# TUMFTM/CamRaDepth

Hardware: AMD Instinct MI355X
Metric: training images/sec at 256x416 bf16 (higher is better)
Workload: dtype bf16; 1 GPU; CamRaDepth base (image+radar) train step, 8x7x256x416 per GPU, bf16 MFMA / fp32 accumulate, diffGradNorm + OneCycleLR, Dropout2d/DropPath on; global_batch=8, parallelism=dp1, hip_graph=True

## Files before the change

camradepth_amd/csrc/norm.hip:

```cpp
#include <stdlib.h>
#include "common.h"

namespace {

constexpr int TPB = 256;
constexpr int U = 4;

struct Map {
  int cg, pl, PL; bool active;
  __device__ Map(int C) {
    int CG = C >> 3;
    PL = TPB / CG;
    if (PL < 1) PL = 1;
    active = threadIdx.x < PL * CG;
    cg = threadIdx.x % CG;
    pl = threadIdx.x / CG;
  }
};

__device__ __forceinline__ void fold_rows(float* sm, int n, int rows) {
  for (int i = threadIdx.x; i < n; i += TPB) {
    float a = sm[i];
    for (int r = 1; r < rows; ++r) a += sm[(long long)r * n + i];
    sm[i] = a;
  }
  __syncthreads();
}

template <int XF>
__global__ __launch_bounds__(TPB) void k_gn_stats(const void* x, int x_f32, int x_ld, long long P, int C, int chunk,
                                                  crd_sum_t* stats, crd_sum_t* chan) {
  extern __shared__ float sm[];
  const int b = blockIdx.y;
  Map m(C);
  float s[8], ss[8];
#pragma unroll
  for (int j = 0; j < 8; ++j) s[j] = ss[j] = 0.f;
  if (m.active) {
    long long p0 = (long long)blockIdx.x * chunk, p1 = p0 + chunk;
    if (p1 > P) p1 = P;
    for (long long p = p0 + m.pl; p < p1; p += (long long)U * m.PL) {
      float v[U][8];
#pragma unroll
      for (int u = 0; u < U; ++u) {
        long long pp = p + (long long)u * m.PL;
        if (pp >= p1) pp = p1 - 1;
        load8t<XF>(x, ((long long)b * P + pp) * x_ld + m.cg * 8, v[u]);
      }
#pragma unroll
      for (int u = 0; u < U; ++u)
        if (p + (long long)u * m.PL < p1) {
#pragma unroll
          for (int j = 0; j < 8; ++j) { s[j] += v[u][j]; ss[j] += v[u][j] * v[u][j]; }
        }
    }
    float4* row = reinterpret_cast<float4*>(sm + (long long)m.pl * 2 * C + m.cg * 16);
#pragma unroll
    for (int j = 0; j < 4; ++j) row[j] = make_float4(s[2 * j], ss[2 * j], s[2 * j + 1], ss[2 * j + 1]);
  }
  __syncthreads();
  fold_rows(sm, 2 * C, m.PL);
  if (chan)
    for (int i = threadIdx.x; i < 2 * C; i += TPB) stat_add(&chan[(long long)b * C * 2 + i], sm[i]);
  if (stats)
    for (int g = threadIdx.x; g < (C >> 4) * 2; g += TPB) {
      int slab = g >> 1, which = g & 1;
      float a = 0.f;
#pragma unroll
      for (int j = 0; j < 16; ++j) a += sm[(slab * 16 + j) * 2 + which];
      stat_add(&stats[((long long)b * (C >> 4) + slab) * 2 + which], a);
    }
}

__global__ __launch_bounds__(TPB) void k_attn_out_residual_stats(const float* x, const float* u, const float* S, const float* bp,
                                                                 const float* dp, long long P, int C, int chunk, float* x1,
                                                                 crd_sum_t* stats) {
  extern __shared__ float sm[];
  const int b = blockIdx.y;
  Map m(C);
  if (m.active) {
    float s[8], ss[8], uu[8], bb[8];
#pragma unroll
    for (int j = 0; j < 8; ++j) s[j] = ss[j] = 0.f;
    const float dps = dp ? dp[b] : 1.f;
    load8(u, (long long)b * C + m.cg * 8, 1, uu);
    load8(bp, m.cg * 8, 1, bb);
    long long p0 = (long long)blockIdx.x * chunk, p1 = p0 + chunk;
    if (p1 > P) p1 = P;
    for (long long p = p0 + m.pl; p < p1; p += (long long)U * m.PL) {
      float v[U][8], sv[U];
#pragma unroll
      for (int q = 0; q < U; ++q) {
        long long pp = p + (long long)q * m.PL;
        if (pp >= p1) pp = p1 - 1;
        load8(x, ((long long)b * P + pp) * C + m.cg * 8, 1, v[q]);
        sv[q] = S[(long long)b * P + pp];
      }
#pragma unroll
      for (int q = 0; q < U; ++q)
        if (p + (long long)q * m.PL < p1) {
#pragma unroll
          for (int j = 0; j < 8; ++j) {
            v[q][j] += dps * bf_round(uu[j] * sv[q] + bb[j]);
            s[j] += v[q][j]; ss[j] += v[q][j] * v[q][j];
          }
          store8_f32(x1, ((long long)b * P + p + (long long)q * m.PL) * C + m.cg * 8, v[q]);
        }
    }
    float4* row = reinterpret_cast<float4*>(sm + (long long)m.pl * 2 * C + m.cg * 16);
#pragma unroll
    for (int j = 0; j < 4; ++j) row[j] = make_float4(s[2 * j], ss[2 * j], s[2 * j + 1], ss[2 * j + 1]);
  }
  __syncthreads();
  fold_rows(sm, 2 * C, m.PL);
  for (int g = threadIdx.x; g < (C >> 4) * 2; g += TPB) {
    int slab = g >> 1, which = g & 1;
    float a = 0.f;
#pragma unroll
    for (int j = 0; j < 16; ++j) a += sm[(slab * 16 + j) * 2 + which];
    stat_add(&stats[((long long)b * (C >> 4) + slab) * 2 + which], a);
  }
}

template <int XF, int YF, int ACT>
__global__ __launch_bounds__(TPB) void k_gn_apply(const void* x, int x_f32, int x_ld, long long P, int C, int chunk,
                                                  const crd_sum_t* stats, int gmul, const float* gamma, const float* beta,
                                                  int act, const float* mask, void* y, int y_ld, int y_f32, float y_inv_scale,
                                                  void* y2, int y2_ld) {
  const int b = blockIdx.y;
  Map m(C);
  if (!m.active) return;
  const int c0 = m.cg * 8;
  long long p0 = (long long)blockIdx.x * chunk, p1 = p0 + chunk;
  if (p1 > P) p1 = P;
  long long p = p0 + m.pl;
  float v[U][8];
  auto load_batch = [&](long long q) {
#pragma unroll
    for (int u = 0; u < U; ++u) {
      long long pp = q + (long long)u * m.PL;
      if (pp >= p1) pp = p1 - 1;
      load8t<XF>(x, ((long long)b * P + pp) * x_ld + c0, v[u]);
    }
  };
  if (p < p1) load_batch(p);
  float ga[8], be[8], mk[8];
  load8(gamma, c0, 1, ga);
  load8(beta, c0, 1, be);
  if (mask) load8(mask, (long long)b * C + c0, 1, mk);
  else {
#pragma unroll
    for (int j = 0; j < 8; ++j) mk[j] = 1.f;
  }
  float mean, rstd;
  const int grp = (c0 >> 4) / gmul;
  gn_mean_rstd(stats + (long long)b * (C >> 4) * 2, grp * gmul, gmul, (float)P * 16.f * gmul, mean, rstd);
#pragma unroll
  for (int j = 0; j < 8; ++j) {
    ga[j] *= rstd;
    be[j] -= mean * ga[j];
  }
  for (bool first = true; p < p1; p += (long long)U * m.PL, first = false) {
    if (!first) load_batch(p);
#pragma unroll
    for (int u = 0; u < U; ++u) {
      const long long pp = p + (long long)u * m.PL;
      if (pp < p1) {
#pragma unroll
        for (int j = 0; j < 8; ++j) {
          float w = v[u][j] * ga[j] + be[j];
          if (ACT == 1) w = gelu_exact(w);
          v[u][j] = w * mk[j];
        }
        if (YF == 3) {
          store8_fp8(y, ((long long)b * P + pp) * y_ld + c0, v[u], y_inv_scale);
          store8_bf16(y2, ((long long)b * P + pp) * y2_ld + c0, v[u]);
        } else if (YF == 2) store8_fp8(y, ((long long)b * P + pp) * y_ld + c0, v[u], y_inv_scale);
        else if (YF) store8_f32(reinterpret_cast<float*>(y), ((long long)b * P + pp) * y_ld + c0, v[u]);
        else store8_bf16(y, ((long long)b * P + pp) * y_ld + c0, v[u]);
      }
    }
  }
}

template <int XF, int DF, int ACT>
__global__ __launch_bounds__(TPB) void k_gn_bwd_reduce(const void* x, int x_f32, int x_ld, const void* dy, int dy_f32,
                                                       int dy_ld, long long P, int C, int Cs, int chunk, const crd_sum_t* stats,
                                                       int gmul, const float* gamma, const float* beta, int act,
                                                       const float* mask, crd_sum_t* r, float* partial) {
  extern __shared__ float sm[];
  const int b = blockIdx.y, cs = blockIdx.z * Cs;
  Map m(Cs);
  if (m.active) {
    const int c0 = cs + m.cg * 8;
    long long p0 = (long long)blockIdx.x * chunk, p1 = p0 + chunk;
    if (p1 > P) p1 = P;
    long long p = p0 + m.pl;
    float v[U][8], d[U][8];
    auto load_batch = [&](long long q) {
#pragma unroll
      for (int u = 0; u < U; ++u) {
        long long pp = q + (long long)u * m.PL;
        if (pp >= p1) pp = p1 - 1;
        load8t<XF>(x, ((long long)b * P + pp) * x_ld + c0, v[u]);
        load8t<DF>(dy, ((long long)b * P + pp) * dy_ld + c0, d[u]);
      }
    };
    if (p < p1) load_batch(p);
    float ga[8], be[8], mk[8], s0[8], s1[8];
    load8(gamma, c0, 1, ga);
    load8(beta, c0, 1, be);
    if (mask) load8(mask, (long long)b * C + c0, 1, mk);
#pragma unroll
    for (int j = 0; j < 8; ++j) {
      if (!mask) mk[j] = 1.f;
      s0[j] = s1[j] = 0.f;
    }
    float mean, rstd;
    const int grp = (c0 >> 4) / gmul;
    gn_mean_rstd(stats + (long long)b * (C >> 4) * 2, grp * gmul, gmul, (float)P * 16.f * gmul, mean, rstd);
    for (bool first = true; p < p1; p += (long long)U * m.PL, first = false) {
      if (!first) load_batch(p);
#pragma unroll
      for (int u = 0; u < U; ++u)
        if (p + (long long)u * m.PL < p1) {
#pragma unroll
          for (int j = 0; j < 8; ++j) {
            float xh = (v[u][j] - mean) * rstd;
            float g = d[u][j] * mk[j];
            if (ACT == 1) g *= gelu_grad(xh * ga[j] + be[j]);
            s0[j] += g; s1[j] += g * xh;
          }
        }
    }
    float4* row = reinterpret_cast<float4*>(sm + (long long)m.pl * 2 * Cs + m.cg * 16);
#pragma unroll
    for (int j = 0; j < 4; ++j) row[j] = make_float4(s0[2 * j], s1[2 * j], s0[2 * j + 1], s1[2 * j + 1]);
  }
  __syncthreads();
  fold_rows(sm, 2 * Cs, m.PL);
  if (partial) {
    float* dst = partial + ((long long)b * gridDim.x + blockIdx.x) * 2 * C + cs * 2;
    for (int i = threadIdx.x; i < 2 * Cs; i += TPB) dst[i] = sm[i];
    return;
  }
  for (int i = threadIdx.x; i < 2 * Cs; i += TPB) {
    const float v = sm[i];
    grad_add(&r[((long long)b * C + cs) * 2 + i], v);
    sm[i] = v * gamma[cs + (i >> 1)];
  }
  __syncthreads();
  const int cpg = 16 * gmul, G = C / cpg, Gs = Cs / cpg;
  crd_sum_t* rg = r + (long long)gridDim.y * C * 2 + ((long long)b * G + cs / cpg) * 2;
  for (int gi = threadIdx.x; gi < 2 * Gs; gi += TPB) {
    const int grp = gi >> 1, which = gi & 1;
    float acc = 0.f;
    for (int c = grp * cpg; c < (grp + 1) * cpg; ++c) acc += sm[c * 2 + which];
    grad_add(&rg[grp * 2 + which], acc);
  }
}

__global__ __launch_bounds__(TPB) void k_gn_bwd_finalize(const float* partial, int nblk, int C, int gmul, const float* gamma,
                                                         crd_sum_t* r, int B) {
  __shared__ float sm[4][64][2];
  const int b = blockIdx.y, c = blockIdx.x * 64 + (threadIdx.x & 63), lane = threadIdx.x >> 6;
  float s0 = 0.f, s1 = 0.f;
  if (c < C)
    for (int k = lane; k < nblk; k += 4) {
      const float* p = partial + ((long long)b * nblk + k) * 2 * C + c * 2;
      s0 += p[0]; s1 += p[1];
    }
  sm[lane][threadIdx.x & 63][0] = s0; sm[lane][threadIdx.x & 63][1] = s1;
  __syncthreads();
  if (lane == 0 && c < C) {
    s0 = sm[0][threadIdx.x][0] + sm[1][threadIdx.x][0] + sm[2][threadIdx.x][0] + sm[3][threadIdx.x][0];
    s1 = sm[0][threadIdx.x][1] + sm[1][threadIdx.x][1] + sm[2][threadIdx.x][1] + sm[3][threadIdx.x][1];
    r[((long long)b * C + c) * 2] = to_fx(s0, GRAD_ONE);
    r[((long long)b * C + c) * 2 + 1] = to_fx(s1, GRAD_ONE);
    const float g = gamma[c];
    sm[0][threadIdx.x][0] = g * s0; sm[0][threadIdx.x][1] = g * s1;
  }
  __syncthreads();
  if (threadIdx.x < 8) {
    const int slab = threadIdx.x >> 1, which = threadIdx.x & 1, c0 = blockIdx.x * 64 + slab * 16;
    if (c0 < C) {
      float a = 0.f;
      for (int j = 0; j < 16; ++j) a += sm[0][slab * 16 + j][which];
      const int cpg = 16 * gmul;
      grad_add(r + (long long)B * C * 2 + ((long long)b * (C / cpg) + c0 / cpg) * 2 + which, a);
    }
  }
}

template <int XF, int DF, int ACT>
__global__ __launch_bounds__(TPB) void k_gn_bwd_apply(const void* x, int x_f32, int x_ld, const void* dy, int dy_f32,
                                                      int dy_ld, long long P, int C, int chunk, const crd_sum_t* stats,
                                                      int gmul, const float* gamma, const float* beta, int act,
                                                      const float* mask, const crd_sum_t* r, float* dgamma, float* dbeta,
                                                      void* dx, int dx_f32, int dx_ld, int dx_acc, int B, void* dx2, int dx2_ld,
                                                      const float* scale2, unsigned char* dx8, int dx8_ld, const float* scale8,
                                                      unsigned* amax8) {
  const int b = blockIdx.y;
  Map m(C);
  const int c0 = m.cg * 8;
  __shared__ float s_amax[TPB / 64];
  const float inv8 = (dx8 && scale8) ? 1.f / fmaxf(*scale8, 1e-30f) : 0.f;
  float amax = 0.f;
  long long p0 = (long long)blockIdx.x * chunk, p1 = p0 + chunk;
  if (p1 > P) p1 = P;
  long long p = p0 + m.pl;
  float v[U][8], d[U][8];
  auto load_batch = [&](long long q) {
#pragma unroll
    for (int u = 0; u < U; ++u) {
      long long pp = q + (long long)u * m.PL;
      if (pp >= p1) pp = p1 - 1;
      load8t<XF>(x, ((long long)b * P + pp) * x_ld + c0, v[u]);
      load8t<DF>(dy, ((long long)b * P + pp) * dy_ld + c0, d[u]);
    }
  };
  if (m.active && p < p1) load_batch(p);
  if (b == 0 && dgamma) {
    for (int c = blockIdx.x * TPB + threadIdx.x; c < C; c += gridDim.x * TPB) {
      const float ob = dbeta[c], og = dgamma[c];
      long long g0, g1;
      sum_samples(r, B, C, c, g0, g1);
      dbeta[c] = ob + (float)g0 * (1.f / GRAD_ONE);
      dgamma[c] = og + (float)g1 * (1.f / GRAD_ONE);
    }
  }
  if (!m.active && !amax8) return;
  if (m.active) {
  float ga[8], be[8], mk[8];
  load8(gamma, c0, 1, ga);
  load8(beta, c0, 1, be);
  if (mask) load8(mask, (long long)b * C + c0, 1, mk);
  else {
#pragma unroll
    for (int j = 0; j < 8; ++j) mk[j] = 1.f;
  }
  const int grp = (c0 >> 4) / gmul;
  const int cpg = 16 * gmul;
  const float inv_m = 1.f / ((float)P * cpg);
  const crd_sum_t* rg = r + (long long)B * C * 2 + ((long long)b * (C / cpg) + grp) * 2;
  const float S1 = grad_get(rg) * inv_m, S2 = grad_get(rg + 1) * inv_m;
  float mean, rstd;
  gn_mean_rstd(stats + (long long)b * (C >> 4) * 2, grp * gmul, gmul, (float)P * cpg, mean, rstd);
  const float sc2 = (dx2 && scale2) ? scale2[b] : 1.f;
  for (bool first = true; p < p1; p += (long long)U * m.PL, first = false) {
    if (!first) load_batch(p);
#pragma unroll
    for (int u = 0; u < U; ++u) {
      const long long pp = p + (long long)u * m.PL;
      if (pp >= p1) continue;
      float o[8];
#pragma unroll
      for (int j = 0; j < 8; ++j) {
        float xh = (v[u][j] - mean) * rstd;
        float g = d[u][j] * mk[j];
        if (ACT == 1) g *= gelu_grad(xh * ga[j] + be[j]);
        o[j] = (ga[j] * g - S1 - xh * S2) * rstd;
      }
      const long long off = ((long long)b * P + pp) * dx_ld + c0;
      if (dx_f32) {
        float* q = reinterpret_cast<float*>(dx);
        if (dx_acc) {
          float w[8];
          load8(dx, off, 1, w);
#pragma unroll
          for (int j = 0; j < 8; ++j) o[j] += w[j];
        }
        store8_f32(q, off, o);
      } else {
        if (dx_acc) {
          float w[8];
          load8(dx, off, 0, w);
#pragma unroll
          for (int j = 0; j < 8; ++j) o[j] += w[j];
        }
        store8_bf16(dx, off, o);
      }
      if (dx8) {
        const uint32_t w0 = pack_bf2(o[0], o[1]), w1 = pack_bf2(o[2], o[3]), w2 = pack_bf2(o[4], o[5]), w3 = pack_bf2(o[6], o[7]);
        const float r[8] = {bf_lo(w0), bf_hi(w0), bf_lo(w1), bf_hi(w1), bf_lo(w2), bf_hi(w2), bf_lo(w3), bf_hi(w3)};
        const float chk = ((r[0] + r[1]) + (r[2] + r[3])) + ((r[4] + r[5]) + (r[6] + r[7]));
        if (!(fabsf(chk) < 3.0e38f)) crd_tu_nonfinite = 1;
#pragma unroll
        for (int j = 0; j < 8; ++j) amax = fmaxf(amax, fabsf(r[j]));
        uint2 q8;
        q8.x = pack_fp8x4(r[0] * inv8, r[1] * inv8, r[2] * inv8, r[3] * inv8);
        q8.y = pack_fp8x4(r[4] * inv8, r[5] * inv8, r[6] * inv8, r[7] * inv8);
        *reinterpret_cast<uint2*>(dx8 + ((long long)b * P + pp) * dx8_ld + c0) = q8;
      }
      if (dx2) {
#pragma unroll
        for (int j = 0; j < 8; ++j) o[j] *= sc2;
        store8_bf16(dx2, ((long long)b * P + pp) * dx2_ld + c0, o);
      }
    }
  }
  }
  if (amax8) {
#pragma unroll
    for (int o_ = 32; o_ > 0; o_ >>= 1) amax = fmaxf(amax, __shfl_xor(amax, o_));
    if ((threadIdx.x & 63) == 0) s_amax[threadIdx.x >> 6] = amax;
    __syncthreads();
    if (threadIdx.x == 0) {
      float a_ = s_amax[0];
      for (int w_ = 1; w_ < TPB / 64; ++w_) a_ = fmaxf(a_, s_amax[w_]);
      if (a_ > 0.f) atomicMax(amax8 + ((blockIdx.x + blockIdx.y * gridDim.x) % CRD_FP8_AMAX_SLOTS), __float_as_uint(a_));
    }
  }
}

inline void grid_for(long long P, int C, int B, dim3& grid, int& chunk, bool reduce = false) {
  int CG = C >> 3;
  int PL = TPB / CG; if (PL < 1) PL = 1;
  long long per_block = (long long)PL * 8;
  long long nblk = (P + per_block - 1) / per_block;
  static int minpix = -1, small = 256;
  if (minpix < 0) {
    minpix = crd_dev_int("CRD_GN_MINPIX", 2);
    small = crd_dev_int("CRD_GN_SMALL", 256);
  }
  if (nblk * B < small && minpix < 8) {
    per_block = (long long)PL * minpix;
    nblk = (P + per_block - 1) / per_block;
  }
  static int cap_r = -1, cap_e = -1;
  if (cap_r < 0) { cap_r = crd_dev_int("CRD_GN_CAP_R", 768); cap_e = crd_dev_int("CRD_GN_CAP_E", 4096); }
  long long cap = (reduce ? cap_r : cap_e) / (B > 0 ? B : 1); if (cap < 1) cap = 1;
  if (nblk > cap) nblk = cap;
  if (nblk < 1) nblk = 1;
  chunk = (int)((P + nblk - 1) / nblk);
  nblk = (P + chunk - 1) / chunk;
  grid = dim3((unsigned)nblk, (unsigned)B);
}

int check_common(const char* name, int x_ld, int x_coff, int C, int x_f32) {
  if (C % 16 != 0 || C > 2048) { crd_set_error("%s: C must be a multiple of 16 and <= 2048 (got %d)", name, C); return CRD_E_UNSUPPORTED; }
  if (x_ld % 8 || x_coff % 8) { crd_set_error("%s: ld/coff must be multiples of 8", name); return CRD_E_INVALID; }
  (void)x_f32;
  return CRD_OK;
}

inline size_t lds_rows(int C) {
  int PL = TPB / (C >> 3); if (PL < 1) PL = 1;
  return (size_t)PL * 2 * C * sizeof(float);
}

inline const void* off_ptr(const void* p, int f32, int coff) {
  return f32 ? (const void*)(reinterpret_cast<const float*>(p) + coff) : (const void*)(reinterpret_cast<const bf16_t*>(p) + coff);
}

}

extern "C" int crd_gn_stats(const void* x, int32_t x_f32, int32_t x_ld, int32_t x_coff, int32_t B, int32_t P, int32_t C,
                            crd_sum_t* stats, crd_sum_t* chan_sums, crd_stream_t stream) {
  CRD_CHECK_ARG(x && (stats || chan_sums), "crd_gn_stats: null pointer");
  int rc = check_common("crd_gn_stats", x_ld, x_coff, C, x_f32);
  if (rc) return rc;
  dim3 grid; int chunk;
  grid_for(P, C, B, grid, chunk, true);
  if (x_f32) hipLaunchKernelGGL(k_gn_stats<1>, grid, dim3(TPB), lds_rows(C), as_stream(stream), off_ptr(x, x_f32, x_coff),
                                x_f32, x_ld, (long long)P, C, chunk, stats, chan_sums);
  else hipLaunchKernelGGL(k_gn_stats<0>, grid, dim3(TPB), lds_rows(C), as_stream(stream), off_ptr(x, x_f32, x_coff),
                          x_f32, x_ld, (long long)P, C, chunk, stats, chan_sums);
  CRD_LAUNCH_CHECK("crd_gn_stats");
  return CRD_OK;
}

extern "C" int crd_attn_out_residual_stats(const float* x, const float* u, const float* S, const float* bp, const float* dp,
                                           int32_t B, int32_t N, int32_t C, float* x1, crd_sum_t* stats, crd_stream_t stream) {
  CRD_CHECK_ARG(x && u && S && bp && x1 && stats, "crd_attn_out_residual_stats: null pointer");
  int rc = check_common("crd_attn_out_residual_stats", C, 0, C, 1);
  if (rc) return rc;
  dim3 grid; int chunk;
  grid_for(N, C, B, grid, chunk, true);
  hipLaunchKernelGGL(k_attn_out_residual_stats, grid, dim3(TPB), lds_rows(C), as_stream(stream), x, u, S, bp, dp, (long long)N, C,
                     chunk, x1, stats);
  CRD_LAUNCH_CHECK("crd_attn_out_residual_stats");
  return CRD_OK;
}

extern "C" int crd_gn_apply(const void* x, int32_t x_f32, int32_t x_ld, int32_t x_coff, int32_t B, int32_t P, int32_t C,
                            const crd_sum_t* stats, int32_t gmul, const float* gamma, const float* beta, int32_t act,
                            const float* mask, void* y, int32_t y_f32, int32_t y_ld, int32_t y_coff, crd_stream_t stream) {
  CRD_CHECK_ARG(x && stats && gamma && beta && y, "crd_gn_apply: null pointer");
  CRD_CHECK_ARG(gmul >= 1 && (C / 16) % gmul == 0, "crd_gn_apply: bad gmul %d for C=%d", gmul, C);
  CRD_CHECK_ARG(y_ld % 8 == 0 && y_coff % 8 == 0, "crd_gn_apply: y_ld/y_coff must be multiples of 8");
  int rc = check_common("crd_gn_apply", x_ld, x_coff, C, x_f32);
  if (rc) return rc;
  dim3 grid; int chunk;
  grid_for(P, C, B, grid, chunk);
  void* yp = y_f32 ? (void*)(reinterpret_cast<float*>(y) + y_coff) : (void*)(reinterpret_cast<bf16_t*>(y) + y_coff);
#define CRD_GN_APPLY(XF, YF, ACT)                                                                                        \
  hipLaunchKernelGGL((k_gn_apply<XF, YF, ACT>), grid, dim3(TPB), 0, as_stream(stream), off_ptr(x, x_f32, x_coff), x_f32, \
                     x_ld, (long long)P, C, chunk, stats, gmul, gamma, beta, act, mask, yp, y_ld, y_f32, 1.f, nullptr, 0)
  const int key = (x_f32 ? 4 : 0) | (y_f32 ? 2 : 0) | (act ? 1 : 0);
  switch (key) {
    case 0: CRD_GN_APPLY(0, 0, 0); break;  case 1: CRD_GN_APPLY(0, 0, 1); break;
    case 2: CRD_GN_APPLY(0, 1, 0); break;  case 3: CRD_GN_APPLY(0, 1, 1); break;
    case 4: CRD_GN_APPLY(1, 0, 0); break;  case 5: CRD_GN_APPLY(1, 0, 1); break;
    case 6: CRD_GN_APPLY(1, 1, 0); break;  default: CRD_GN_APPLY(1, 1, 1); break;
  }
#undef CRD_GN_APPLY
  CRD_LAUNCH_CHECK("crd_gn_apply");
  return CRD_OK;
}

extern "C" int crd_gn_apply_fp8(const void* x, int32_t x_f32, int32_t x_ld, int32_t x_coff, int32_t B, int32_t P, int32_t C,
                                const crd_sum_t* stats, int32_t gmul, const float* gamma, const float* beta, int32_t act,
                                const float* mask, void* y_fp8, int32_t y_ld, int32_t y_coff, float y_scale, void* y_bf16,
                                int32_t yb_ld, int32_t yb_coff, crd_stream_t stream) {
  CRD_CHECK_ARG(x && stats && gamma && beta && y_fp8 && y_scale > 0.f, "crd_gn_apply_fp8: null pointer / bad scale");
  CRD_CHECK_ARG(gmul >= 1 && (C / 16) % gmul == 0, "crd_gn_apply_fp8: bad gmul %d for C=%d", gmul, C);
  CRD_CHECK_ARG(y_ld % 8 == 0 && y_coff % 8 == 0 && yb_ld % 8 == 0 && yb_coff % 8 == 0, "crd_gn_apply_fp8: ld/coff must be multiples of 8");
  int rc = check_common("crd_gn_apply_fp8", x_ld, x_coff, C, x_f32);
  if (rc) return rc;
  dim3 grid; int chunk;
  grid_for(P, C, B, grid, chunk);
  void* yp = reinterpret_cast<unsigned char*>(y_fp8) + y_coff;
  void* y2 = y_bf16 ? (void*)(reinterpret_cast<bf16_t*>(y_bf16) + yb_coff) : nullptr;
#define CRD_GN_APPLY8(XF, YF, ACT)                                                                                       \
  hipLaunchKernelGGL((k_gn_apply<XF, YF, ACT>), grid, dim3(TPB), 0, as_stream(stream), off_ptr(x, x_f32, x_coff), x_f32, \
                     x_ld, (long long)P, C, chunk, stats, gmul, gamma, beta, act, mask, yp, y_ld, 0, 1.f / y_scale, y2, yb_ld)
  switch ((x_f32 ? 4 : 0) | (y2 ? 2 : 0) | (act ? 1 : 0)) {
    case 0: CRD_GN_APPLY8(0, 2, 0); break;  case 1: CRD_GN_APPLY8(0, 2, 1); break;
    case 2: CRD_GN_APPLY8(0, 3, 0); break;  case 3: CRD_GN_APPLY8(0, 3, 1); break;
    case 4: CRD_GN_APPLY8(1, 2, 0); break;  case 5: CRD_GN_APPLY8(1, 2, 1); break;
    case 6: CRD_GN_APPLY8(1, 3, 0); break;  default: CRD_GN_APPLY8(1, 3, 1); break;
  }
#undef CRD_GN_APPLY8
  CRD_LAUNCH_CHECK("crd_gn_apply_fp8");
  return CRD_OK;
}

extern "C" int crd_gn_bwd_reduce(const void* x, int32_t x_f32, int32_t x_ld, int32_t x_coff, const void* dy, int32_t dy_f32,
                                 int32_t dy_ld, int32_t dy_coff, int32_t B, int32_t P, int32_t C, const crd_sum_t* stats,
                                 int32_t gmul, const float* gamma, const float* beta, int32_t act, const float* mask,
                                 crd_sum_t* r, float* scratch, int64_t scratch_capacity, crd_stream_t stream) {
  CRD_CHECK_ARG(x && dy && stats && gamma && beta && r, "crd_gn_bwd_reduce: null pointer");
  CRD_CHECK_ARG(gmul >= 1 && (C / 16) % gmul == 0, "crd_gn_bwd_reduce: bad gmul");
  CRD_CHECK_ARG(dy_ld % 8 == 0 && dy_coff % 8 == 0, "crd_gn_bwd_reduce: dy_ld/dy_coff must be multiples of 8");
  int rc = check_common("crd_gn_bwd_reduce", x_ld, x_coff, C, x_f32);
  if (rc) return rc;
  dim3 grid; int chunk;
  int S = 1;
  static int slicing = -1;
  if (slicing < 0) slicing = crd_dev_int("CRD_GN_RED_SLICES", 1);
  if (slicing && !scratch && C >= 256) {
    const int cpg = 16 * gmul;
    for (int s_ = 8; s_ > 1; s_ >>= 1)
      if (C % s_ == 0 && (C / s_) % cpg == 0 && (C / s_) % 8 == 0 && C / s_ >= 64) { S = s_; break; }
  }
  const int Cs = C / S;
  grid_for(P, Cs, B * S, grid, chunk, true);
  grid = dim3(grid.x, (unsigned)B, (unsigned)S);
  float* part = (scratch && (long long)B * grid.x * 2 * C <= scratch_capacity && grid.x > 1) ? scratch : nullptr;
#define CRD_GN_RED(XF, DF, ACT)                                                                                              \
  hipLaunchKernelGGL((k_gn_bwd_reduce<XF, DF, ACT>), grid, dim3(TPB), lds_rows(Cs), as_stream(stream),                     \
                     off_ptr(x, x_f32, x_coff), x_f32, x_ld, off_ptr(dy, dy_f32, dy_coff), dy_f32, dy_ld, (long long)P, C, \
                     Cs, chunk, stats, gmul, gamma, beta, act, mask, r, part)
  switch ((x_f32 ? 4 : 0) | (dy_f32 ? 2 : 0) | (act ? 1 : 0)) {
    case 0: CRD_GN_RED(0, 0, 0); break;  case 1: CRD_GN_RED(0, 0, 1); break;
    case 2: CRD_GN_RED(0, 1, 0); break;  case 3: CRD_GN_RED(0, 1, 1); break;
    case 4: CRD_GN_RED(1, 0, 0); break;  case 5: CRD_GN_RED(1, 0, 1); break;
    case 6: CRD_GN_RED(1, 1, 0); break;  default: CRD_GN_RED(1, 1, 1); break;
  }
#undef CRD_GN_RED
  if (part)
    hipLaunchKernelGGL(k_gn_bwd_finalize, dim3(cdiv(C, 64), B), dim3(TPB), 0, as_stream(stream), scratch, (int)grid.x, C, gmul,
                       gamma, r, B);
  CRD_LAUNCH_CHECK("crd_gn_bwd_reduce");
  return CRD_OK;
}

static int gn_bwd_apply_impl(const void* x, int32_t x_f32, int32_t x_ld, int32_t x_coff, const void* dy, int32_t dy_f32,
                             int32_t dy_ld, int32_t dy_coff, int32_t B, int32_t P, int32_t C, const crd_sum_t* stats,
                             int32_t gmul, const float* gamma, const float* beta, int32_t act, const float* mask,
                             const crd_sum_t* r, float* dgamma, float* dbeta, void* dx, int32_t dx_f32, int32_t dx_ld,
                             int32_t dx_coff, int32_t dx_accumulate, void* dx2, int32_t dx2_ld, const float* scale2,
                             void* dx8, int32_t dx8_ld, int32_t dx8_coff, const float* scale8, uint32_t* amax8, crd_stream_t stream) {
  unsigned char* dx8p = dx8 ? reinterpret_cast<unsigned char*>(dx8) + dx8_coff : nullptr;
  CRD_CHECK_ARG(x && dy && stats && gamma && beta && r && dx, "crd_gn_bwd_apply: null pointer");
  CRD_CHECK_ARG(!dx2 || dx2_ld % 8 == 0, "crd_gn_bwd_apply: dx2_ld must be a multiple of 8");
  CRD_CHECK_ARG((dgamma == nullptr) == (dbeta == nullptr), "crd_gn_bwd_apply: dgamma and dbeta go together");
  CRD_CHECK_ARG(gmul >= 1 && (C / 16) % gmul == 0, "crd_gn_bwd_apply: bad gmul");
  CRD_CHECK_ARG(dy_ld % 8 == 0 && dy_coff % 8 == 0 && dx_ld % 8 == 0 && dx_coff % 8 == 0,
                "crd_gn_bwd_apply: dy/dx ld/coff must be multiples of 8");
  int rc = check_common("crd_gn_bwd_apply", x_ld, x_coff, C, x_f32);
  if (rc) return rc;
  dim3 grid; int chunk;
  grid_for(P, C, B, grid, chunk);
  void* dxp = dx_f32 ? (void*)(reinterpret_cast<float*>(dx) + dx_coff) : (void*)(reinterpret_cast<bf16_t*>(dx) + dx_coff);
#define CRD_GN_BAP(XF, DF, ACT)                                                                                              \
  hipLaunchKernelGGL((k_gn_bwd_apply<XF, DF, ACT>), grid, dim3(TPB), 0, as_stream(stream), off_ptr(x, x_f32, x_coff), x_f32, \
                     x_ld, off_ptr(dy, dy_f32, dy_coff), dy_f32, dy_ld, (long long)P, C, chunk, stats, gmul, gamma, beta,  \
                     act, mask, r, dgamma, dbeta, dxp, dx_f32, dx_ld, dx_accumulate, B, dx2, dx2_ld, scale2, dx8p, dx8_ld, scale8,  \
                     amax8)
  switch ((x_f32 ? 4 : 0) | (dy_f32 ? 2 : 0) | (act ? 1 : 0)) {
    case 0: CRD_GN_BAP(0, 0, 0); break;  case 1: CRD_GN_BAP(0, 0, 1); break;
    case 2: CRD_GN_BAP(0, 1, 0); break;  case 3: CRD_GN_BAP(0, 1, 1); break;
    case 4: CRD_GN_BAP(1, 0, 0); break;  case 5: CRD_GN_BAP(1, 0, 1); break;
    case 6: CRD_GN_BAP(1, 1, 0); break;  default: CRD_GN_BAP(1, 1, 1); break;
  }
#undef CRD_GN_BAP
  CRD_LAUNCH_CHECK("crd_gn_bwd_apply");
  return CRD_OK;
}

extern "C" int crd_gn_bwd_apply(const void* x, int32_t x_f32, int32_t x_ld, int32_t x_coff, const void* dy, int32_t dy_f32,
                                int32_t dy_ld, int32_t dy_coff, int32_t B, int32_t P, int32_t C, const crd_sum_t* stats,
                                int32_t gmul, const float* gamma, const float* beta, int32_t act, const float* mask,
                                const crd_sum_t* r, float* dgamma, float* dbeta, void* dx, int32_t dx_f32, int32_t dx_ld,
                                int32_t dx_coff, int32_t dx_accumulate, void* dx2, int32_t dx2_ld, const float* scale2,
                                crd_stream_t stream) {
  return gn_bwd_apply_impl(x, x_f32, x_ld, x_coff, dy, dy_f32, dy_ld, dy_coff, B, P, C, stats, gmul, gamma, beta, act, mask, r, dgamma, dbeta,
                           dx, dx_f32, dx_ld, dx_coff, dx_accumulate, dx2, dx2_ld, scale2, nullptr, 0, 0, nullptr, nullptr, stream);
}

extern "C" int crd_gn_bwd_apply_fp8(const void* x, int32_t x_f32, int32_t x_ld, int32_t x_coff, const void* dy, int32_t dy_f32,
                                    int32_t dy_ld, int32_t dy_coff, int32_t B, int32_t P, int32_t C, const crd_sum_t* stats,
                                    int32_t gmul, const float* gamma, const float* beta, int32_t act, const float* mask,
                                    const crd_sum_t* r, float* dgamma, float* dbeta, void* dx, int32_t dx_ld, int32_t dx_coff,
                                    void* dx_fp8, int32_t dx8_ld, int32_t dx8_coff, const float* scale_dev, uint32_t* amax_slots,
                                    crd_stream_t stream) {
  CRD_CHECK_ARG(dx_fp8 && scale_dev && amax_slots && dx8_ld % 8 == 0 && dx8_coff % 8 == 0,
                "crd_gn_bwd_apply_fp8: the e4m3 copy needs its buffer, a device scale and the amax slots (ld / coff multiples of 8)");
  return gn_bwd_apply_impl(x, x_f32, x_ld, x_coff, dy, dy_f32, dy_ld, dy_coff, B, P, C, stats, gmul, gamma, beta, act, mask, r, dgamma, dbeta,
                           dx, 0, dx_ld, dx_coff, 0, nullptr, 0, nullptr, dx_fp8, dx8_ld, dx8_coff, scale_dev, amax_slots, stream);
}
```

camradepth_amd/lib.py:

```python
import ctypes as C
import os
import struct

import torch

_HERE = os.path.dirname(os.path.abspath(__file__))
LIB_PATH = os.environ.get("CRD_LIB") or os.path.join(_HERE, "libcamradepth_hip.so")


class CrdError(RuntimeError):
    pass


class ConvDesc(C.Structure):
    _fields_ = [
        ("x", C.c_void_p), ("x_ld", C.c_int32), ("x_coff", C.c_int32),
        ("B", C.c_int32), ("IH", C.c_int32), ("IW", C.c_int32), ("Cin", C.c_int32),
        ("w", C.c_void_p), ("Cout", C.c_int32), ("KH", C.c_int32), ("KW", C.c_int32),
        ("stride", C.c_int32), ("pad", C.c_int32), ("OH", C.c_int32), ("OW", C.c_int32),
        ("gather_mode", C.c_int32),
        ("y", C.c_void_p), ("y_ld", C.c_int32), ("y_coff", C.c_int32), ("y_f32", C.c_int32),
        ("out_mode", C.c_int32), ("patch_k", C.c_int32), ("patch_c", C.c_int32),
        ("bias", C.c_void_p), ("bias_bstride", C.c_int32), ("act", C.c_int32),
        ("res", C.c_void_p), ("res_ld", C.c_int32), ("res_scale", C.c_void_p),
        ("accumulate", C.c_int32), ("stats", C.c_void_p),
        ("stats_partial", C.c_void_p), ("stats_partial_capacity", C.c_int64),
        ("red_x", C.c_void_p), ("red_x_ld", C.c_int32), ("red_gmul", C.c_int32), ("red_act", C.c_int32),
        ("red_x_f32", C.c_int32), ("red_stats", C.c_void_p), ("red_gamma", C.c_void_p), ("red_beta", C.c_void_p),
        ("red_r", C.c_void_p), ("chan_sums", C.c_void_p),
    ]


class GnInput(C.Structure):
    _fields_ = [("x_f32", C.c_int32), ("gmul", C.c_int32), ("stats", C.c_void_p), ("gamma", C.c_void_p), ("beta", C.c_void_p),
                ("act", C.c_int32), ("xn_ld", C.c_int32), ("xn", C.c_void_p)]


class GnBwdInput(C.Structure):
    _fields_ = [("gx", C.c_void_p), ("gx_f32", C.c_int32), ("gx_ld", C.c_int32), ("gmul", C.c_int32), ("act", C.c_int32),
                ("stats", C.c_void_p), ("gamma", C.c_void_p), ("beta", C.c_void_p), ("mask", C.c_void_p), ("r", C.c_void_p),
                ("dx", C.c_void_p), ("dx_ld", C.c_int32), ("dgamma", C.c_void_p), ("dbeta", C.c_void_p)]


class WgradDesc(C.Structure):
    _fields_ = [
        ("x", C.c_void_p), ("x_ld", C.c_int32), ("x_coff", C.c_int32),
        ("B", C.c_int32), ("IH", C.c_int32), ("IW", C.c_int32), ("Cin", C.c_int32),
        ("dy", C.c_void_p), ("dy_ld", C.c_int32), ("dy_coff", C.c_int32),
        ("OH", C.c_int32), ("OW", C.c_int32), ("Cout", C.c_int32),
        ("KH", C.c_int32), ("KW", C.c_int32), ("stride", C.c_int32), ("pad", C.c_int32),
        ("dw", C.c_void_p), ("dbias", C.c_void_p), ("dw_partials", C.c_void_p), ("dw_partial_capacity", C.c_int32), ("wg_budget", C.c_int32),
    ]


class WgradGroupInfo(C.Structure):
    _fields_ = [("n_problems", C.c_int32), ("n_items", C.c_int32 * 4), ("item_offset", C.c_int32 * 4), ("bytes", C.c_int64)]


class PackEntry(C.Structure):
    _fields_ = [
        ("src", C.c_void_p), ("dst_fwd", C.c_void_p), ("dst_dgrad", C.c_void_p), ("dst_scatter", C.c_void_p),
        ("cmap", C.c_void_p),
        ("Cout", C.c_int32), ("Cin_ref", C.c_int32), ("taps", C.c_int32), ("Cin_pad", C.c_int32),
        ("Cout_pad", C.c_int32), ("dst_f32", C.c_int32),
        ("dgrad_ld", C.c_int32), ("dgrad_coff", C.c_int32), ("dgrad_row0", C.c_int32), ("dgrad_rows", C.c_int32),
    ]


class MlpDesc(C.Structure):
    _fields_ = [(n, C.c_void_p) for n in ("x1", "x1_stats", "norm_gamma", "norm_beta", "w_fc1", "b_fc1", "norm1_gamma", "norm1_beta",
                                          "w9", "b_dw", "norm2_gamma", "norm2_beta", "w_fc2", "xn", "h1", "h2", "h3", "h1_stats",
                                          "h2_stats", "fc2_partials")] + \
               [(n, C.c_int32) for n in ("B", "H", "W", "C", "hidden")]


class UnpackEntry(C.Structure):
    _fields_ = [
        ("src", C.c_void_p), ("dst", C.c_void_p), ("cmap", C.c_void_p),
        ("Cout", C.c_int32), ("Cin_ref", C.c_int32), ("taps", C.c_int32), ("Cin_pad", C.c_int32),
        ("replicas", C.c_int32), ("src_sum", C.c_int32), ("replica_stride", C.c_int64),
    ]


class DgnDesc(C.Structure):
    _fields_ = [(n, C.c_void_p) for n in ("p", "g", "exp_avg", "exp_avg_sq", "prev_grad", "exp_grad_norm", "factor", "parts", "seg_off",
                                          "blk2seg", "blk2chunk", "active", "hp_dev", "gate", "clip", "ema")] + \
               [("parts_stride", C.c_int64), ("n_tensors", C.c_int32), ("n_blocks", C.c_int32)] + \
               [(n, C.c_float) for n in ("lr", "beta1", "beta2", "eps", "weight_decay")] + \
               [("step", C.c_int32), ("max_norm", C.c_float), ("ema_decay", C.c_float),
                ("ema_warmup", C.c_int32), ("ema_n", C.c_int32), ("ema_base", C.c_int32)]


_lib = None
ABI_VERSION = 13


def load():
    global _lib
    if _lib is not None:
        return _lib
    if not os.path.exists(LIB_PATH):
        raise CrdError(f"{LIB_PATH} is missing: run `python -m camradepth_amd.build` (hipcc, gfx950). "
                       "camradepth_amd has no CPU fallback.")
    lib = C.CDLL(LIB_PATH)
    lib.crd_last_error.restype = C.c_char_p
    lib.crd_arch.restype = C.c_char_p
    lib.crd_version.restype = C.c_int
    if lib.crd_version() != ABI_VERSION:
        raise CrdError(f"{LIB_PATH} was built for ABI version {lib.crd_version()}, this binding is version {ABI_VERSION}: rebuild it "
                       "(python -m camradepth_amd.build)")
    missing = [n for n in EXPORTS if not hasattr(lib, n)]
    if missing:
        raise CrdError(f"{LIB_PATH} lacks symbols {missing}: rebuild it (python -m camradepth_amd.build)")
    for name, sig in _SIGS.items():
        fn = getattr(lib, name)
        fn.restype = C.c_int
        fn.argtypes = [_CT[ch] for ch in sig]
    if os.environ.get("CRD_DEV_SWITCHES") == "1":
        if os.environ.get("CRD_TUNE_REGE") is not None:
            lib.crd_tune_igemm_reg_epilogue(int(os.environ["CRD_TUNE_REGE"]))
        if os.environ.get("CRD_TUNE_NARROW") is not None:
            lib.crd_tune_pw_narrow(int(os.environ["CRD_TUNE_NARROW"]))
    _lib = lib
    return lib


_SIGS = {
    "crd_conv_igemm": "pp", "crd_conv_igemm_route": "ppi", "crd_gn_conv": "ppp", "crd_gn_conv2": "ppppp", "crd_gn_bwd_conv": "ppp", "crd_pw_narrow_supported": "iii", "crd_tune_pw_narrow": "i", "crd_conv3x3_fp8": "ppfp", "crd_amax_bf16": "pliiipp", "crd_quant_fp8": "pliiipiifp",
    "crd_weight_quant_fp8": "piiiippp", "crd_conv3x3_fp8_dgrad": "pppp", "crd_gn_bwd_apply_fp8": "piiipiiiiiipippipppppiipiippp",
    "crd_fp8_scale_update": "ppifip", "crd_quant_fp8_dev": "pliiipiipp", "crd_tune_conv3x3_small_grid": "i", "crd_tune_igemm_reg_epilogue": "i", "crd_conv_wgrad": "pp", "crd_conv_wgrad_splits": "p", "crd_conv_wgrad_route": "ppi", "crd_wgrad_group_build": "piplp", "crd_conv_wgrad_grouped": "ppp",
    "crd_gn_stats": "piiiiiippp", "crd_gn_apply": "piiiiiipippipPiiip".replace("P", "p"),
    "crd_gn_bwd_reduce": "piiipiiiiiipippippplp", "crd_gn_bwd_apply": "piiipiiiiiipippipppppiiiipipp",
    "crd_dwconv3x3": "piiiippipppippppppp", "crd_dwconv3x3_wgrad": "ppiiiipipippp",
    "crd_attn_scores": "ppiiiiifppp", "crd_attn_scores_fp8": "ppiiiiffppp", "crd_attn_fwd": "ppiiiiifpppppppppp", "crd_attn_xbar": "ppppiiipp", "crd_attn_xbar_proj": "pppppiiippp", "crd_attn_vec_bwd": "ppiiifppp", "crd_attn_out_residual": "pppppiiipp", "crd_attn_out_residual_stats": "pppppiiippp",
    "crd_attn_out_bwd": "ppppiiipppp", "crd_attn_out_bwd_blocks": "iii", "crd_attn_out_bwd_gn": "ppppiiippppppppppp", "crd_attn_scores_bwd": "ppppiiiiifpppp", "crd_attn_bwd": "ppppiiiiifpppppifppp", "crd_attn_scores_bwd_partials": "iiiii", "crd_sum_partials_bf16": "pilplp", "crd_gsum_to_bf16": "pplp",
    "crd_attn_bwd_fused_supported": "iiiii", "crd_attn_bwd_fused": "ppppppp" "iiiii" "f" "ppppp" "ppppppp" "p", "crd_attn_dk_fold": "pilpl" "pp" "iii" "f" "pp" "p",
    "crd_bicubic2x": "piiiiiipiip", "crd_bicubic2x_fp8": "piiiiiipiifpiip", "crd_gn_apply_fp8": "piiiiiipippippiifpiip", "crd_bicubic2x_bwd": "piiiiiipiiip",
    "crd_input_grad": "ppppiiiiiipp",
    "crd_nchw_to_pm": "piiiipiiip", "crd_pm_to_nchw": "piiiiiiipp", "crd_seg_argmax": "piiiiipiiip", "crd_scale_f32": "pplfp",
    "crd_slice_copy": "piipiiliip", "crd_f32_to_bf16_rows": "pipiiliplpiip", "crd_dropout_masks": "ppiiLpp", "crd_sigmoid_bwd": "pplp", "crd_head_conv2_fwd": "pppiiippiip", "crd_head_conv2_bwd": "ppiippiiippip", "crd_head_conv2_bwd_data": "ppiippiiipp", "crd_head_conv2_wgrad": "ppiipiiipip",
    "crd_weight_pack": "pilp", "crd_wgrad_unpack": "pilip",
    "crd_assemble_input": "pppiiifpp", "crd_gt_pyramid": "piiifppppp",
    "crd_augment_draw": "ppiiiiifffffffiLLp", "crd_augment_lut": "piipp", "crd_augment_assemble": "pppppppiiiiifppppp",
    "crd_augment_gather": "ppppiiiiiippppp", "crd_gt_pyramid_from_full": "piiipppp",
    "crd_radar_project": "pppiipppipiiiffpppppppp", "crd_radar_rasterize": "ppppppppiipiiiiiplppp",
    "crd_lidar_project": "pppiippppippipppipiiiffLLpppppppppp", "crd_lidar_ground_truth": "pppppppppiipiiiiipppipLplpppp",
    "crd_depth_unproject": "piiiiipipiiLLLipppppp", "crd_point_cloud": "piiiiipipiiLLLipppipplpppppp",
    "crd_bev_grid": "ppppiiipiLLLiiLLiiiplppppppp",
    "crd_occupancy_update": "pppiiipipipiiiiLiLLLLiiiiiipppppplpppppp",
    "crd_distance_field": "piiiiiippplppppp", "crd_field_paths": "pppiipLpppiiiiiippppppp",
    "crd_nav_field": "piiippipLiiipppp", "crd_nav_paths": "ppiipLppiiipppppp",
    "crd_map_objects": "piiiiiiipLplpppppp",
    "crd_track_objects": "pppp" "iiiii" "LLLL" "ii" "ppppppppp" "p",
    "crd_match_scan": "ppp" "iii" "pipi" "iii" "LLLL" "i" "ppp" "ii" "p" "il" "pl" "ppppppp" "p",
    "crd_viz_range": "piiiiipplpp", "crd_viz_draw": "piiiippffipiiffipllp", "crd_seg_labels": "piiiipp",
    "crd_camera_frontend": "piiiilliiippip",
    "crd_resize_nearest_u8":"piiiipiip", "crd_resize_labels_nearest": "piiiipiip", "crd_seg_confusion": "ppiilppp",
    "crd_masked_l1_fwd": "pplpp", "crd_test_metrics": "ppilffpp", "crd_depth_eval": "ppilfffipp", "crd_masked_l1_bwd": "pplppfpp", "crd_ce_fwd": "ppiilpp",
    "crd_ce_focal_bwd": "ppiilppfpp",
    "crd_masked_dist_fwd": "pplpp", "crd_masked_dist_bwd": "pplppfipp", "crd_masked_berhu_max": "pplppp",
    "crd_masked_berhu": "pplppLppfpp", "crd_smoothness_fwd": "ppiiiipp", "crd_smoothness_bwd": "ppiiiippfpp",
    "crd_diffgradnorm_norm": "pp", "crd_diffgradnorm_commit": "pp", "crd_diffgradnorm_step": "pp",
    "crd_mlp_fused_supported": "iiii", "crd_mlp_fwd": "pp", "crd_mlp_reduce": "pipppiiipppp",
    "crd_nonfinite_status": "ip", "crd_nonfinite_capture": "pp",
    "crd_swap_f32": "pplp",
}
_CT = {"p": C.c_void_p, "i": C.c_int32, "l": C.c_int64, "L": C.c_uint64, "f": C.c_float}
EXPORTS = list(_SIGS)


STAT_FRAC_BITS, GRAD_FRAC_BITS = 20, 44
SUM_DTYPE = torch.int64
EVAL_FRAC_BITS = (0, 32, 26, 24, 24, 36, 33, 31, 40, 0, 0, 0)
EVAL_MAX_BINS = 64
AUGMENT_WORDS, AUGMENT_STREAM = 8, 0xA0761D6478BD642F
AUGMENT_GAMMA, AUGMENT_BRIGHTNESS, AUGMENT_COLOUR = 1, 2, 4


def stat_value(t):
    return t.double() * 2.0 ** -STAT_FRAC_BITS


def grad_value(t):
    return t.double() * 2.0 ** -GRAD_FRAC_BITS


def nonfinite(reset=True):
    rc = load().crd_nonfinite_status(1 if reset else 0, stream())
    if rc < 0:
        check(rc, "crd_nonfinite_status")
    return rc == 1


def nonfinite_clear():
    check(load().crd_nonfinite_status(2, stream()), "crd_nonfinite_status")


def stat_checked(acc):
    v = stat_value(acc)
    if nonfinite(reset=False):
        v = torch.full_like(v, float("nan"))
    return v


def f64_bits(x):
    return struct.unpack("<Q", struct.pack("<d", float(x)))[0]


def check(rc, what=""):
    if rc != 0:
        msg = load().crd_last_error().decode()
        raise CrdError(f"{what} failed with status {rc}: {msg}")


def conv_route(desc):
    buf = C.create_string_buffer(96)
    check(load().crd_conv_igemm_route(C.byref(desc), buf, len(buf)), "crd_conv_igemm_route")
    return buf.value.decode()


def wgrad_route(desc):
    buf = C.create_string_buffer(96)
    check(load().crd_conv_wgrad_route(C.byref(desc), buf, len(buf)), "crd_conv_wgrad_route")
    return buf.value.decode()


def stream():
    return C.c_void_p(torch.cuda.current_stream().cuda_stream)


def ptr(t):
    return None if t is None else C.c_void_p(t.data_ptr())
```

include/camradepth_hip.h:

```cpp
#ifndef CAMRADEPTH_HIP_H
#define CAMRADEPTH_HIP_H

#include <stdint.h>

#ifdef __cplusplus
extern "C" {
#endif

typedef void* crd_stream_t;

#define CRD_OK 0
#define CRD_E_INVALID (-1)
#define CRD_E_UNSUPPORTED (-2)
#define CRD_E_LAUNCH (-3)

typedef int64_t crd_sum_t;
#define CRD_STAT_FRAC_BITS 20
#define CRD_GRAD_FRAC_BITS 44
int crd_nonfinite_status(int32_t reset, crd_stream_t stream);
int crd_nonfinite_capture(int32_t* window_flag, crd_stream_t stream);

const char* crd_last_error(void);
#define CRD_ABI_VERSION 13
int crd_version(void);
const char* crd_arch(void);

typedef struct {
  const void* x;
  int32_t x_ld, x_coff;
  int32_t B, IH, IW, Cin;
  const void* w;
  int32_t Cout, KH, KW, stride, pad;
  int32_t OH, OW;
  int32_t gather_mode;
  void* y;
  int32_t y_ld, y_coff;
  int32_t y_f32;
  int32_t out_mode;
  int32_t patch_k, patch_c;
  const float* bias;
  int32_t bias_bstride;
  int32_t act;
  const float* res;
  int32_t res_ld;
  const float* res_scale;
  int32_t accumulate;
  crd_sum_t* stats;
  float* stats_partial;
  int64_t stats_partial_capacity;
  const void* red_x;
  int32_t red_x_ld, red_gmul, red_act, red_x_f32;
  const crd_sum_t* red_stats;
  const float* red_gamma;
  const float* red_beta;
  crd_sum_t* red_r;
  crd_sum_t* chan_sums;
} crd_conv_desc;

int crd_conv_igemm(const crd_conv_desc* d, crd_stream_t stream);
int crd_conv_igemm_route(const crd_conv_desc* d, char* label, int32_t capacity);

typedef struct {
  int32_t x_f32;
  int32_t gmul;
  const crd_sum_t* stats;
  const float* gamma;
  const float* beta;
  int32_t act;
  int32_t xn_ld;
  void* xn;
} crd_gn_input;
int crd_gn_conv(const crd_conv_desc* d, const crd_gn_input* n, crd_stream_t stream);
int crd_gn_conv2(const crd_conv_desc* d0, const crd_gn_input* n0, const crd_conv_desc* d1, const crd_gn_input* n1, crd_stream_t stream);
typedef struct {
  const void* gx; int32_t gx_f32, gx_ld;
  int32_t gmul, act;
  const crd_sum_t* stats;
  const float* gamma; const float* beta;
  const float* mask;
  const crd_sum_t* r;
  void* dx; int32_t dx_ld;
  float* dgamma; float* dbeta;
} crd_gn_bwd_input;
int crd_gn_bwd_conv(const crd_conv_desc* d, const crd_gn_bwd_input* n, crd_stream_t stream);
int crd_pw_narrow_supported(int32_t Cin, int32_t Cout, int32_t pixels);
int crd_tune_pw_narrow(int32_t on);
int crd_tune_conv3x3_small_grid(int workgroups);
int crd_tune_igemm_reg_epilogue(int32_t on);

int crd_conv3x3_fp8(const crd_conv_desc* d, const float* w_scales, float x_scale, crd_stream_t stream);
int crd_amax_bf16(const void* x, int64_t rows, int32_t ld, int32_t coff, int32_t C, float* amax, crd_stream_t stream);
int crd_quant_fp8(const void* x, int64_t rows, int32_t ld, int32_t coff, int32_t C, void* y, int32_t y_ld, int32_t y_coff,
                  float scale, crd_stream_t stream);
int crd_gn_apply_fp8(const void* x, int32_t x_f32, int32_t x_ld, int32_t x_coff, int32_t B, int32_t P, int32_t C, const crd_sum_t* stats,
                     int32_t gmul, const float* gamma, const float* beta, int32_t act, const float* mask, void* y_fp8, int32_t y_ld,
                     int32_t y_coff, float y_scale, void* y_bf16, int32_t yb_ld, int32_t yb_coff, crd_stream_t stream);
int crd_bicubic2x_fp8(const void* x, int32_t x_ld, int32_t x_coff, int32_t B, int32_t H, int32_t W, int32_t C, void* y_fp8,
                      int32_t y_ld, int32_t y_coff, float y_scale, void* y_bf16, int32_t yb_ld, int32_t yb_coff, crd_stream_t stream);
int crd_weight_quant_fp8(const void* w_bf16, int32_t Cout, int32_t taps, int32_t Cin, int32_t Cin_out, void* w_fp8, float* scales,
                         crd_stream_t stream);

int crd_conv3x3_fp8_dgrad(const crd_conv_desc* d, const float* w_scales, const float* x_scale_dev, crd_stream_t stream);
#define CRD_FP8_AMAX_SLOTS 64
int crd_gn_bwd_apply_fp8(const void* x, int32_t x_f32, int32_t x_ld, int32_t x_coff, const void* dy, int32_t dy_f32,
                         int32_t dy_ld, int32_t dy_coff, int32_t B, int32_t P, int32_t C, const crd_sum_t* stats,
                         int32_t gmul, const float* gamma, const float* beta, int32_t act, const float* mask,
                         const crd_sum_t* r, float* dgamma, float* dbeta, void* dx, int32_t dx_ld, int32_t dx_coff,
                         void* dx_fp8, int32_t dx8_ld, int32_t dx8_coff, const float* scale_dev, uint32_t* amax_slots,
                         crd_stream_t stream);
int crd_fp8_scale_update(uint32_t* amax_slots, float* scales, int32_t n, float margin, int32_t keep_slots, crd_stream_t stream);
int crd_quant_fp8_dev(const void* x, int64_t rows, int32_t ld, int32_t coff, int32_t C, void* y, int32_t y_ld, int32_t y_coff,
                      const float* scale_dev, crd_stream_t stream);

typedef struct {
  const void* x; int32_t x_ld, x_coff; int32_t B, IH, IW, Cin;
  const void* dy; int32_t dy_ld, dy_coff; int32_t OH, OW, Cout;
  int32_t KH, KW, stride, pad;
  crd_sum_t* dw;
  crd_sum_t* dbias;
  float* dw_partials;
  int32_t dw_partial_capacity;
  int32_t wg_budget;
} crd_wgrad_desc;

int crd_conv_wgrad(const crd_wgrad_desc* d, crd_stream_t stream);
int crd_conv_wgrad_splits(const crd_wgrad_desc* d);
int crd_conv_wgrad_route(const crd_wgrad_desc* d, char* label, int32_t capacity);

typedef struct crd_wgrad_group_info {
  int32_t n_problems;
  int32_t n_items[4];
  int32_t item_offset[4];
  int64_t bytes;
} crd_wgrad_group_info;
int crd_wgrad_group_build(const crd_wgrad_desc* descs, int32_t n, void* host_table, int64_t capacity,
                          crd_wgrad_group_info* info);
int crd_conv_wgrad_grouped(const void* dev_table, const crd_wgrad_group_info* info, crd_stream_t stream);

int crd_gn_stats(const void* x, int32_t x_f32, int32_t x_ld, int32_t x_coff, int32_t B, int32_t P, int32_t C,
                 crd_sum_t* stats, crd_sum_t* chan_sums, crd_stream_t stream);

int crd_gn_apply(const void* x, int32_t x_f32, int32_t x_ld, int32_t x_coff, int32_t B, int32_t P, int32_t C,
                 const crd_sum_t* stats, int32_t gmul, const float* gamma, const float* beta, int32_t act,
                 const float* mask, void* y, int32_t y_f32, int32_t y_ld, int32_t y_coff, crd_stream_t stream);

int crd_gn_bwd_reduce(const void* x, int32_t x_f32, int32_t x_ld, int32_t x_coff, const void* dy, int32_t dy_f32,
                      int32_t dy_ld, int32_t dy_coff, int32_t B, int32_t P, int32_t C, const crd_sum_t* stats,
                      int32_t gmul, const float* gamma, const float* beta, int32_t act, const float* mask,
                      crd_sum_t* r, float* scratch, int64_t scratch_capacity, crd_stream_t stream);
int crd_gn_bwd_apply(const void* x, int32_t x_f32, int32_t x_ld, int32_t x_coff, const void* dy, int32_t dy_f32,
                     int32_t dy_ld, int32_t dy_coff, int32_t B, int32_t P, int32_t C, const crd_sum_t* stats,
                     int32_t gmul, const float* gamma, const float* beta, int32_t act, const float* mask,
                     const crd_sum_t* r, float* dgamma, float* dbeta, void* dx, int32_t dx_f32, int32_t dx_ld,
                     int32_t dx_coff, int32_t dx_accumulate, void* dx2, int32_t dx2_ld, const float* scale2,
                     crd_stream_t stream);


int crd_dwconv3x3(const void* x, int32_t B, int32_t H, int32_t W, int32_t C, const float* w9, const float* bias,
                  int32_t flip, void* y, crd_sum_t* stats, const crd_sum_t* in_stats, int32_t in_gmul, const float* in_gamma,
                  const float* in_beta, const void* red_x, const crd_sum_t* red_stats, const float* red_gamma, crd_sum_t* red_r,
                  crd_stream_t stream);
int crd_dwconv3x3_wgrad(const void* x, const void* dy, int32_t B, int32_t H, int32_t W, int32_t C, crd_sum_t* dw10,
                        int32_t replicas, const crd_sum_t* in_stats, int32_t in_gmul, const float* in_gamma,
                        const float* in_beta, crd_stream_t stream);

typedef struct {
  const float* x1; const crd_sum_t* x1_stats; const float* norm_gamma; const float* norm_beta;
  const void* w_fc1; const float* b_fc1; const float* norm1_gamma; const float* norm1_beta;
  const float* w9; const float* b_dw; const float* norm2_gamma; const float* norm2_beta;
  const void* w_fc2;
  void* xn; void* h1; void* h2; void* h3;
  crd_sum_t* h1_stats; crd_sum_t* h2_stats;
  float* fc2_partials;
  int32_t B, H, W, C, hidden;
} crd_mlp_desc;
int crd_mlp_fused_supported(int32_t H, int32_t W, int32_t C, int32_t hidden);
int crd_mlp_fwd(const crd_mlp_desc* d, crd_stream_t stream);
int crd_mlp_reduce(const float* fc2_partials, int32_t slabs, const float* x1, const float* b_fc2, const float* dp, int32_t B,
                   int32_t N, int32_t C, float* x2, crd_sum_t* stats, crd_sum_t* chan_sums, crd_stream_t stream);

int crd_attn_scores(const void* q, const void* k, int32_t B, int32_t N, int32_t M, int32_t heads, int32_t d,
                    float scale, float* S, int16_t* idx, crd_stream_t stream);
int crd_attn_scores_fp8(const void* q8, const void* k8, int32_t B, int32_t N, int32_t M, int32_t heads, float qk_scale, float scale,
                        float* ssum, int16_t* idx, crd_stream_t stream);
int crd_attn_fwd(const void* q, const void* k, int32_t B, int32_t N, int32_t M, int32_t heads, int32_t d, float scale,
                 float* S, int16_t* idx, const crd_sum_t* chan_sums, const crd_sum_t* stats, const float* gamma, const float* beta,
                 const void* w_fwd, void* xbar, float* u, crd_stream_t stream);
int crd_attn_xbar(const crd_sum_t* chan_sums, const crd_sum_t* stats, const float* gamma, const float* beta, int32_t B,
                  int32_t N, int32_t C, void* xbar, crd_stream_t stream);
int crd_attn_xbar_proj(const crd_sum_t* chan_sums, const crd_sum_t* stats, const float* gamma, const float* beta, const void* w_fwd,
                       int32_t B, int32_t N, int32_t C, void* xbar, float* u, crd_stream_t stream);
int crd_attn_vec_bwd(const crd_sum_t* t, const void* w_dgrad, int32_t B, int32_t C, int32_t Cpad, float inv_n, void* tb, float* es,
                     crd_stream_t stream);
int crd_attn_out_residual(const float* x, const float* u, const float* S, const float* bp, const float* dp,
                          int32_t B, int32_t N, int32_t C, float* x1, crd_stream_t stream);
int crd_attn_out_residual_stats(const float* x, const float* u, const float* S, const float* bp, const float* dp,
                                int32_t B, int32_t N, int32_t C, float* x1, crd_sum_t* stats, crd_stream_t stream);
int crd_attn_out_bwd(const float* dx1, const float* u, const float* S, const float* dp, int32_t B, int32_t N,
                     int32_t C, crd_sum_t* t, crd_sum_t* dbp_rows, float* dS, crd_stream_t stream);
int crd_attn_out_bwd_gn(float* dx1, const float* u, const float* S, const float* dp, int32_t B, int32_t N, int32_t C,
                        crd_sum_t* t, crd_sum_t* dbp_rows, float* dS, const float* x, const void* dxn, const crd_sum_t* stats,
                        const float* gamma, const crd_sum_t* r, float* dgamma, float* dbeta, crd_stream_t stream);
int crd_attn_out_bwd_blocks(int32_t B, int32_t N, int32_t C);
int crd_attn_scores_bwd_partials(int32_t B, int32_t N, int32_t M, int32_t heads, int32_t d);
int crd_attn_scores_bwd(const void* q, const void* k, const float* dS, const int16_t* idx, int32_t B, int32_t N,
                        int32_t M, int32_t heads, int32_t d, float scale, void* dq, crd_sum_t* dk, float* dk_partials,
                        crd_stream_t stream);
int crd_attn_bwd(const void* q, const void* k, const float* dS, const int16_t* idx, int32_t B, int32_t N, int32_t M,
                 int32_t heads, int32_t d, float scale, void* dq, crd_sum_t* dk, float* dk_partials, const crd_sum_t* t,
                 const void* w_dgrad, int32_t Cpad, float inv_n, void* tb, float* es, crd_stream_t stream);
int crd_sum_partials_bf16(const float* part, int32_t replicas, int64_t replica_stride, void* dst, int64_t n,
                          crd_stream_t stream);
int crd_attn_bwd_fused_supported(int32_t B, int32_t N, int32_t M, int32_t heads, int32_t d);
int crd_attn_bwd_fused(float* dx1, const float* u, const float* S, const float* dp, const void* q, const void* k, const int16_t* idx,
                       int32_t B, int32_t N, int32_t M, int32_t heads, int32_t d, float scale, crd_sum_t* t, crd_sum_t* dbp_rows,
                       float* dS, void* dq, float* dk_partials, const float* x, const void* dxn, const crd_sum_t* stats,
                       const float* gamma, const crd_sum_t* r, float* dgamma, float* dbeta, crd_stream_t stream);
int crd_attn_dk_fold(const float* part, int32_t replicas, int64_t replica_stride, void* dst, int64_t n, const crd_sum_t* t,
                     const void* w_dgrad, int32_t B, int32_t C, int32_t Cpad, float inv_n, void* tb, float* es, crd_stream_t stream);
int crd_gsum_to_bf16(const crd_sum_t* src, void* dst, int64_t n, crd_stream_t stream);

int crd_bicubic2x(const void* x, int32_t x_ld, int32_t x_coff, int32_t B, int32_t H, int32_t W, int32_t C, void* y,
                  int32_t y_ld, int32_t y_coff, crd_stream_t stream);
int crd_bicubic2x_bwd(const void* dy, int32_t dy_ld, int32_t dy_coff, int32_t B, int32_t H, int32_t W, int32_t C,
                      void* dx, int32_t dx_ld, int32_t dx_coff, int32_t accumulate, crd_stream_t stream);

int crd_input_grad(const void* draw, const void* wpe, const void* dcb_depth, const void* dcb_seg, int32_t dcb_ld, int32_t col0,
                   int32_t B, int32_t H, int32_t W, int32_t Cin, float* dx, crd_stream_t stream);

int crd_nchw_to_pm(const float* x, int32_t B, int32_t C, int32_t H, int32_t W, void* y, int32_t y_ld, int32_t y_coff,
                   int32_t Cpad, crd_stream_t stream);
int crd_pm_to_nchw(const void* x, int32_t x_f32, int32_t x_ld, int32_t x_coff, int32_t B, int32_t C, int32_t H,
                   int32_t W, float* y, crd_stream_t stream);
int crd_seg_argmax(const void* logits, int32_t ld, int32_t B, int32_t P, int32_t C, int32_t num_classes, void* y,
                   int32_t y_f32, int32_t y_ld, int32_t y_coff, crd_stream_t stream);
int crd_scale_f32(const float* src, float* dst, int64_t n, float scale, crd_stream_t stream);
int crd_slice_copy(const void* src, int32_t s_ld, int32_t s_coff, void* dst, int32_t d_ld, int32_t d_coff,
                   int64_t rows, int32_t C, int32_t accumulate, crd_stream_t stream);
int crd_f32_to_bf16_rows(const float* src, int32_t s_ld, void* dst, int32_t d_ld, int32_t d_coff, int64_t rows,
                         int32_t C, const float* scale, int64_t rows_per_sample, const void* add, int32_t add_ld,
                         int32_t add_coff, crd_stream_t stream);
int crd_head_conv2_fwd(const void* a, const float* w, const float* bias, int32_t B, int32_t H, int32_t W, float* depth,
                       void* copy, int32_t copy_ld, int32_t copy_coff, crd_stream_t stream);
int crd_head_conv2_bwd(const float* gd, const void* add, int32_t add_ld, int32_t add_coff, const void* a, const float* w,
                       int32_t B, int32_t H, int32_t W, void* dz, crd_sum_t* dw_rows, int32_t replicas, crd_stream_t stream);
int crd_head_conv2_bwd_data(const float* gd, const void* add, int32_t add_ld, int32_t add_coff, const void* a, const float* w,
                            int32_t B, int32_t H, int32_t W, void* dz, crd_stream_t stream);
int crd_head_conv2_wgrad(const float* gd, const void* add, int32_t add_ld, int32_t add_coff, const void* a, int32_t B, int32_t H,
                         int32_t W, crd_sum_t* dw_rows, int32_t replicas, crd_stream_t stream);
int crd_sigmoid_bwd(const void* a, void* da, int64_t n, crd_stream_t stream);

typedef struct {
  const float* src;
  void* dst_fwd;
  void* dst_dgrad;
  void* dst_scatter;
  const int32_t* cmap;
  int32_t Cout, Cin_ref, taps, Cin_pad, Cout_pad;
  int32_t dst_f32;
  int32_t dgrad_ld, dgrad_coff, dgrad_row0, dgrad_rows;
} crd_pack_entry;
int crd_weight_pack(const crd_pack_entry* table_dev, int32_t n, int64_t max_elems, crd_stream_t stream);
typedef struct {
  const void* src;
  float* dst;
  const int32_t* cmap;
  int32_t Cout, Cin_ref, taps, Cin_pad;
  int32_t replicas;
  int32_t src_sum;
  int64_t replica_stride;
} crd_unpack_entry;
int crd_wgrad_unpack(const crd_unpack_entry* table_dev, int32_t n, int64_t max_elems, int32_t accumulate,
                     crd_stream_t stream);

int crd_dropout_masks(float* out, const float* keep, int32_t rows, int32_t cols, uint64_t seed, uint64_t* counter,
                      crd_stream_t stream);

int crd_assemble_input(const void* img_u8, const float* radar, const float* rad_vel, int32_t B, int32_t H, int32_t W,
                       float max_depth, float* out, crd_stream_t stream);
int crd_gt_pyramid(const float* depth, int32_t B, int32_t H, int32_t W, float max_depth, float* full, float* half,
                   float* quarter, float* eighth, crd_stream_t stream);
int crd_resize_nearest_u8(const void* src, int32_t B, int32_t SH, int32_t SW, int32_t C, void* dst, int32_t DH, int32_t DW,
                          crd_stream_t stream);
int crd_resize_labels_nearest(const void* src_u8, int32_t B, int32_t SH, int32_t SW, int32_t rows, int64_t* dst, int32_t DH,
                              int32_t DW, crd_stream_t stream);

#define CRD_AUGMENT_WORDS 8
#define CRD_AUGMENT_STREAM 0xA0761D6478BD642Full
#define CRD_AUGMENT_GAMMA 1
#define CRD_AUGMENT_BRIGHTNESS 2
#define CRD_AUGMENT_COLOUR 4
int crd_augment_draw(int32_t* params, float* lut, int32_t B, int32_t H, int32_t W, int32_t h, int32_t w, float p_flip,
                     float gamma_lo, float gamma_hi, float brightness_lo, float brightness_hi, float colour_lo, float colour_hi,
                     int32_t enable, uint64_t seed, uint64_t counter, crd_stream_t stream);
int crd_augment_lut(const int32_t* params, int32_t B, int32_t enable, float* lut, crd_stream_t stream);
int crd_augment_assemble(const void* img_u8, const float* radar, const float* rad_vel, const float* depth, const void* seg_u8,
                         const int32_t* params, const float* lut, int32_t B, int32_t H, int32_t W, int32_t h, int32_t w,
                         float max_depth, float* out, float* gt_full, int64_t* final_seg, int64_t* inter_seg,
                         crd_stream_t stream);
int crd_augment_gather(const float* image, const float* gt_full, const int64_t* seg, const int32_t* params, int32_t B, int32_t C,
                       int32_t H, int32_t W, int32_t h, int32_t w, float* image_out, float* gt_out, int64_t* seg_out,
                       int64_t* inter_out, crd_stream_t stream);
int crd_gt_pyramid_from_full(const float* full, int32_t B, int32_t H, int32_t W, float* half, float* quarter, float* eighth,
                             crd_stream_t stream);

int crd_radar_project(const double* points, const int32_t* sweep_index, const int32_t* frame_offsets, int32_t B, int32_t n_points,
                      const double* cam1_from_sensor, const double* cam2_from_sensor, const double* lags, int32_t n_sweeps,
                      const double* K, int32_t k_stride, int32_t im_h, int32_t im_w, float min_distance, float min_z, double* x1,
                      double* y1, double* depth1, double* x2, double* y2, double* v_comp, uint8_t* valid, crd_stream_t stream);
int crd_radar_rasterize(const double* x1, const double* y1, const double* depth1, const double* x2, const double* y2,
                        const double* v_comp, const uint8_t* valid, const int32_t* frame_offsets, int32_t B, int32_t n_points,
                        const double* K, int32_t k_stride, int32_t im_h, int32_t im_w, int32_t downsample_scale, int32_t y_cutoff,
                        void* workspace, int64_t workspace_bytes, float* radar, float* rad_vel, crd_stream_t stream);

int crd_lidar_project(const double* points, const int32_t* sweep_index, const int32_t* frame_offsets, int32_t B, int32_t n_points,
                      const double* cam1_from_sensor, const double* cam2_from_sensor, const double* car_z_from_sensor,
                      const int32_t* sweep_boxes, int32_t n_sweeps, const double* box_entries, const int32_t* box_id, int32_t n_entries,
                      const double* cam1_from_box, const double* cam2_from_box, const uint8_t* vehicle, int32_t n_boxes,
                      const double* K, int32_t k_stride, int32_t im_h, int32_t im_w, float min_distance, float min_z,
                      uint64_t h_min_f64_bits, uint64_t h_max_f64_bits, double* x1, double* y1, double* depth1, double* x2, double* y2,
                      uint8_t* low_h, uint8_t* in_box, uint8_t* valid, int32_t* box_entry, crd_stream_t stream);
int crd_lidar_ground_truth(const double* x1, const double* y1, const double* depth1, const double* x2, const double* y2,
                           const uint8_t* low_h, const uint8_t* in_box, const uint8_t* valid, const int32_t* frame_offsets, int32_t B,
                           int32_t n_points, const double* K, int32_t k_stride, int32_t im_h, int32_t im_w, int32_t downsample_scale,
                           int32_t y_cutoff, const uint8_t* seg, const double* corners, const int32_t* corner_offsets, int32_t n_boxes,
                           const float* flow_im, uint64_t thres_f64_bits, void* workspace, int64_t workspace_bytes, float* gt,
                           float* depth, uint8_t* msk_lh, crd_stream_t stream);

int crd_depth_unproject(const float* depth, int32_t B, int32_t im_h, int32_t im_w, int32_t downsample_scale, int32_t y_cutoff,
                        const double* K, int32_t k_stride, const double* out_from_cam, int32_t t_stride, int32_t encoding,
                        uint64_t max_depth_f64_bits, uint64_t min_range_f64_bits, uint64_t max_range_f64_bits, int32_t skip_empty,
                        const uint8_t* mask, const uint8_t* labels, const uint8_t* keep, float* points, uint8_t* valid,
                        crd_stream_t stream);
#define CRD_CLOUD_TILE 1024
int crd_point_cloud(const float* depth, int32_t B, int32_t im_h, int32_t im_w, int32_t downsample_scale, int32_t y_cutoff,
                    const double* K, int32_t k_stride, const double* out_from_cam, int32_t t_stride, int32_t encoding,
                    uint64_t max_depth_f64_bits, uint64_t min_range_f64_bits, uint64_t max_range_f64_bits, int32_t skip_empty,
                    const uint8_t* mask, const uint8_t* labels, const uint8_t* keep, int32_t stride, const uint8_t* image,
                    void* workspace, int64_t workspace_bytes, float* xyz, uint8_t* rgb, uint8_t* label, int32_t* pixel,
                    int32_t* frame_offsets, crd_stream_t stream);

int crd_bev_grid(const float* xyz, const uint8_t* valid, const uint8_t* label, const int32_t* frame_offsets, int32_t rows_per_frame,
                 int32_t B, int32_t n_rows, const double* grid_from_points, int32_t t_stride, uint64_t x_min_f64_bits,
                 uint64_t y_min_f64_bits, uint64_t cell_f64_bits, int32_t nx, int32_t ny, uint64_t z_lo_f64_bits, uint64_t z_hi_f64_bits,
                 int32_t min_points, int32_t flip_x, int32_t flip_y, void* workspace, int64_t workspace_bytes, int32_t* count, float* z_max,
                 float* z_min, int32_t* top_index, uint8_t* top_label, uint8_t* occupancy, crd_stream_t stream);

int crd_occupancy_update(const float* xyz, const uint8_t* valid, const int32_t* frame_offsets, int32_t rows_per_frame, int32_t B,
                         int32_t n_rows, const double* map_from_points, int32_t t_stride, const double* sensor, int32_t sensor_stride,
                         const double* centre, int32_t centre_stride, int32_t M, int32_t nx, int32_t ny, uint64_t cell_f64_bits,
                         int32_t n_bins, uint64_t max_range_f64_bits, uint64_t z_floor_f64_bits, uint64_t z_lo_f64_bits,
                         uint64_t z_hi_f64_bits, int32_t min_points, int32_t l_occ, int32_t l_free, int32_t l_max, int32_t occupied_at,
                         int32_t free_at, int16_t* map, int64_t* prev_origin, int64_t* cur_origin, int32_t* initialised, int32_t* status,
                         void* workspace, int64_t workspace_bytes, int16_t* log_odds, uint8_t* state, uint8_t* evidence, float* value,
                         int64_t* origin, crd_stream_t stream);

int crd_distance_field(const uint8_t* state, int32_t M, int32_t nx, int32_t ny, int32_t sources, int32_t max_cells, int32_t unknown_cost,
                       const float* clear_table, const uint8_t* cost_table, void* workspace, int64_t workspace_bytes, int32_t* dist2,
                       int32_t* nearest, float* clearance, uint8_t* cost, crd_stream_t stream);
int crd_field_paths(const double* xy, const int32_t* n_poses, const int32_t* path_map, int32_t K, int32_t P, const int64_t* origin,
                    uint64_t cell_f64_bits, const uint8_t* state, const int32_t* dist2, const uint8_t* cost, int32_t M, int32_t nx,
                    int32_t ny, int32_t max_cells, int32_t blocked_at, int32_t outside_blocks, int32_t* first_blocked, uint8_t* max_cost,
                    int32_t* min_dist2, int32_t* n_outside, int32_t* n_unknown, int32_t* pose_cell, crd_stream_t stream);

int crd_nav_field(const uint8_t* cost, int32_t M, int32_t nx, int32_t ny, const double* goals, const int32_t* n_goals, int32_t G,
                  const int64_t* origin, uint64_t cell_f64_bits, int32_t neutral, int32_t blocked_at, int32_t max_rounds, int32_t* togo,
                  uint8_t* next, int32_t* info, crd_stream_t stream);
int crd_nav_paths(const double* starts, const int32_t* path_map, int32_t K, int32_t P, const int64_t* origin, uint64_t cell_f64_bits,
                  const int32_t* togo, const uint8_t* next, int32_t M, int32_t nx, int32_t ny, int32_t* cells, double* xy, int32_t* n_cells,
                  int32_t* start_togo, int32_t* status, crd_stream_t stream);

int crd_map_objects(const uint8_t* state, int32_t M, int32_t nx, int32_t ny, int32_t sources, int32_t connectivity, int32_t min_cells,
                    int32_t max_objects, const int64_t* origin, uint64_t cell_f64_bits, void* workspace, int64_t workspace_bytes,
                    int32_t* label, int32_t* objects, int64_t* sums, double* centre, int32_t* info, crd_stream_t stream);

int crd_track_objects(const int32_t* objects, const double* centre, const int32_t* objects_info, const int64_t* origin, int32_t M, int32_t N,
                      int32_t T, int32_t nx, int32_t ny, uint64_t cell_f64_bits, uint64_t gate_f64_bits, uint64_t alpha_f64_bits,
                      uint64_t beta_f64_bits, int32_t confirm_hits, int32_t max_misses, int64_t* ids, int32_t* tracks, double* pos, double* vel,
                      int64_t* box, int64_t* next_id, int32_t* track_of, int64_t* id_of, int32_t* info, crd_stream_t stream);

int crd_match_scan(const float* xyz, const uint8_t* valid, const int32_t* frame_offsets, int32_t rows_per_frame, int32_t B, int32_t n_rows,
                   const double* map_from_points, int32_t t_stride, const double* sensor, int32_t sensor_stride, int32_t M, int32_t nx,
                   int32_t ny, uint64_t cell_f64_bits, uint64_t max_range_f64_bits, uint64_t z_lo_f64_bits, uint64_t z_hi_f64_bits,
                   int32_t min_points, const int16_t* map, const int64_t* cur_origin, const int32_t* initialised, int32_t n_xy,
                   int32_t n_theta, const double* rot, int32_t min_cells, int64_t min_score, void* workspace, int64_t workspace_bytes,
                   double* pose, int32_t* pick, int64_t* score, int64_t* prior_score, int32_t* n_cells, int32_t* status, int64_t* scores,
                   crd_stream_t stream);

#define CRD_VIZ_TILE 1024
#define CRD_VIZ_FLOAT 0
#define CRD_VIZ_LABELS 1
#define CRD_VIZ_NONE 0
#define CRD_VIZ_PASTE 1
#define CRD_VIZ_BLEND 2
#define CRD_VIZ_IMAGE 3
int crd_viz_range(const void* src, int32_t kind, int32_t B, int32_t h, int32_t w, int32_t dilate, float* dilated, void* workspace,
                  int64_t workspace_bytes, float* range, crd_stream_t stream);
int crd_viz_draw(const void* src, int32_t kind, int32_t B, int32_t h, int32_t w, const uint8_t* table, const float* range, float vmin,
                 float vmax, int32_t bad_rgb, const uint8_t* image, int32_t image_bgr, int32_t mode, float alpha, float beta,
                 int32_t grey, uint8_t* out, int64_t out_row_pitch, int64_t out_frame_pitch, crd_stream_t stream);
int crd_seg_labels(const float* logits, int32_t B, int32_t C, int32_t h, int32_t w, uint8_t* labels, crd_stream_t stream);

int crd_camera_frontend(const uint8_t* frames, int32_t B, int32_t im_h, int32_t im_w, int32_t channels, int64_t row_pitch,
                        int64_t frame_pitch, int32_t swap_rb, int32_t downsample_scale, int32_t y_cutoff, uint8_t* image_u8, float* x,
                        int32_t x_channels, crd_stream_t stream);

int crd_masked_l1_fwd(const float* pred, const float* target, int64_t n, crd_sum_t* acc, crd_stream_t stream);
int crd_test_metrics(const float* pred, const float* gt, int32_t frames, int64_t n, float max_depth, float max_distance,
                     crd_sum_t* acc, crd_stream_t stream);
int crd_seg_confusion(const float* logits, const int64_t* labels, int32_t frames, int32_t C, int64_t HW, int64_t* confmat,
                      int64_t* out_of_range, crd_stream_t stream);
#define CRD_EVAL_COLUMNS 12
#define CRD_EVAL_MAX_BINS 64
static const int CRD_EVAL_FRAC_BITS[CRD_EVAL_COLUMNS] = {0, 32, 26, 24, 24, 36, 33, 31, 40, 0, 0, 0};
int crd_depth_eval(const float* pred, const float* gt, int32_t frames, int64_t n, float max_depth, float min_depth, float bin_width,
                   int32_t n_bins, crd_sum_t* acc , crd_stream_t stream);
int crd_masked_l1_bwd(const float* pred, const float* target, int64_t n, const crd_sum_t* acc, const float* gout,
                      float gmul, float* dpred, crd_stream_t stream);
int crd_ce_fwd(const float* logits, const int64_t* labels, int32_t B, int32_t C, int64_t HW, crd_sum_t* acc,
               crd_stream_t stream);
int crd_ce_focal_bwd(const float* logits, const int64_t* labels, int32_t B, int32_t C, int64_t HW, const crd_sum_t* acc,
                     const float* gout, float gmul, float* dlogits, crd_stream_t stream);

int crd_masked_dist_fwd(const float* pred, const float* target, int64_t n, crd_sum_t* acc, crd_stream_t stream);
int crd_masked_dist_bwd(const float* pred, const float* target, int64_t n, const crd_sum_t* acc, const float* gout,
                        float gmul, int32_t mode, float* dpred, crd_stream_t stream);
int crd_masked_berhu_max(const float* pred, const float* target, int64_t n, crd_sum_t* acc, int32_t* maxbits, crd_stream_t stream);
int crd_masked_berhu(const float* pred, const float* target, int64_t n, const crd_sum_t* acc, const int32_t* maxbits,
                     uint64_t thresh_f64_bits, crd_sum_t* loss, const float* gout, float gmul, float* dpred, crd_stream_t stream);
int crd_smoothness_fwd(const float* pred, const float* image, int32_t B, int32_t C, int32_t H, int32_t W, crd_sum_t* acc,
                       crd_stream_t stream);
int crd_smoothness_bwd(const float* pred, const float* image, int32_t B, int32_t C, int32_t H, int32_t W, const crd_sum_t* acc,
                       const float* gout, float gmul, float* dpred, crd_stream_t stream);

typedef struct crd_dgn_desc {
  float* p; const float* g; float* exp_avg; float* exp_avg_sq; float* prev_grad; float* exp_grad_norm; float* factor;
  float* parts;
  const int64_t* seg_off; const int32_t* blk2seg; const int32_t* blk2chunk;
  const uint8_t* active;
  const float* hp_dev;
  int32_t* gate;
  float* clip;
  float* ema;
  int64_t parts_stride;
  int32_t n_tensors, n_blocks;
  float lr, beta1, beta2, eps, weight_decay;
  int32_t step;
  float max_norm;
  float ema_decay;
  int32_t ema_warmup, ema_n, ema_base;
} crd_dgn_desc;
int crd_diffgradnorm_norm(const crd_dgn_desc* d, crd_stream_t stream);
int crd_diffgradnorm_commit(const crd_dgn_desc* d, crd_stream_t stream);
int crd_diffgradnorm_step(const crd_dgn_desc* d, crd_stream_t stream);
int crd_swap_f32(float* a, float* b, int64_t n, crd_stream_t stream);

#ifdef __cplusplus
}
#endif
#endif
```

Baseline: 465.1 images/s.

## Software-pipeline GroupNorm kernels with rotating loads and specialized backward-apply variants

Rewrites the GroupNorm apply, backward-reduce and backward-apply kernels around a streaming loop that issues the next pixel's load right after consuming the current one. It uses byte-offset pointer walkers instead of 64-bit index math and adds occupancy hints to launch bounds. Backward apply is templated on output format, accumulate, dual-output and fp8 modes so runtime branches disappear, and a new grid sizing helper changes chunking. The aim is to hide memory latency with fewer registers. The cost is more kernel instantiations, and the scheduling barriers may constrain the compiler.

After: 477.4 images/s (median of 6 runs). 1.03x the previous value.

```diff
diff --git a/camradepth_amd/csrc/norm.hip b/camradepth_amd/csrc/norm.hip
--- a/camradepth_amd/csrc/norm.hip
+++ b/camradepth_amd/csrc/norm.hip
@@ -1,4 +1,5 @@
 #include <stdlib.h>
+#include <utility>
 #include "common.h"
 
 namespace {
@@ -122,8 +123,117 @@
   }
 }
 
+template <int F32> struct Gran;
+template <> struct Gran<0> {
+  uint4 q;
+  __device__ __forceinline__ void load(const char* p) { q = *reinterpret_cast<const uint4*>(p); }
+  __device__ __forceinline__ void get(float (&v)[8]) const { unpack8(q, v); }
+};
+template <> struct Gran<1> {
+  float4 a, b;
+  __device__ __forceinline__ void load(const char* p) {
+    a = reinterpret_cast<const float4*>(p)[0]; b = reinterpret_cast<const float4*>(p)[1];
+  }
+  __device__ __forceinline__ void get(float (&v)[8]) const {
+    v[0] = a.x; v[1] = a.y; v[2] = a.z; v[3] = a.w; v[4] = b.x; v[5] = b.y; v[6] = b.z; v[7] = b.w;
+  }
+};
+struct Walk {
+  char* base; unsigned off, step;
+  __device__ Walk(const void* tensor, int elem_bytes, long long first_row, int ld, int c0, int pl, int PL)
+      : base(reinterpret_cast<char*>(const_cast<void*>(tensor)) + first_row * ld * elem_bytes),
+        off((unsigned)(pl * ld + c0) * elem_bytes), step((unsigned)(PL * ld) * elem_bytes) {}
+  __device__ __forceinline__ char* next() { char* r = base + off; off += step; return r; }
+};
+
+template <int NU, class Req>
+__device__ __forceinline__ void stream_first(int q, int n, int PL, Req&& request) {
+  if (NU * PL <= n) {
+#pragma unroll
+    for (int u = 0; u < NU; ++u) request(u);
+  } else {
+#pragma unroll
+    for (int u = 0; u < NU; ++u)
+      if (q + u * PL < n) request(u);
+  }
+}
+template <int NU, class Req, class Take, class Work>
+__device__ __forceinline__ void stream_pixels(int q, int n, int PL, Req&& request, Take&& take, Work&& work) {
+  const int step = NU * PL;
+  int done = 0;
+#pragma nounroll
+  for (; done + 2 * step <= n; done += step) {
+#pragma unroll
+    for (int u = 0; u < NU; ++u) {
+      take(u);
+      request(u);
+      work();
+      __builtin_amdgcn_sched_barrier(0);
+    }
+  }
+  q += done;
+  if (done + step <= n) {
+#pragma unroll
+    for (int u = 0; u < NU; ++u) {
+      take(u);
+      if (q + u * PL + step < n) request(u);
+      work();
+    }
+    q += step;
+    done += step;
+  }
+  if (done < n) {
+#pragma unroll
+    for (int u = 0; u < NU; ++u)
+      if (q + u * PL < n) {
+        take(u);
+        work();
+      }
+  }
+}
+
+template <int ACT>
+__device__ __forceinline__ float gn_fwd_elem(float v, float ga, float be, float mk) {
+  float w = v * ga + be;
+  if (ACT == 1) w = gelu_exact(w);
+  return w * mk;
+}
+__device__ __forceinline__ float gn_xhat(float v, float mean, float rstd) { return (v - mean) * rstd; }
+template <int ACT>
+__device__ __forceinline__ float gn_bwd_g(float xh, float d, float ga, float be, float mk) {
+  float g = d * mk;
+  if (ACT == 1) g *= gelu_grad(xh * ga + be);
+  return g;
+}
+__device__ __forceinline__ float gn_bwd_dx(float xh, float g, float ga, float S1, float S2, float rstd) {
+  return (ga * g - S1 - xh * S2) * rstd;
+}
+__device__ __forceinline__ float add_rounded(float a, float b) {
+#pragma clang fp contract(off)
+  return a + b;
+}
+
+#ifndef CRD_GN_U_APPLY
+#define CRD_GN_U_APPLY 4
+#endif
+#ifndef CRD_GN_U_BWD
+#define CRD_GN_U_BWD 2
+#endif
+#ifndef CRD_GN_U_RED
+#define CRD_GN_U_RED 2
+#endif
+constexpr int U_APPLY = CRD_GN_U_APPLY, U_BWD = CRD_GN_U_BWD, U_RED = CRD_GN_U_RED;
+#ifndef CRD_GN_WAVES
+#define CRD_GN_WAVES 4
+#endif
+constexpr int GN_WAVES = CRD_GN_WAVES, GN_AHEAD_BYTES = 96;
+constexpr int gn_form_slots(int slots, int bytes_per_slot) {
+  while (slots > 1 && (slots / 2) * bytes_per_slot >= GN_AHEAD_BYTES) slots /= 2;
+  return slots;
+}
+
 template <int XF, int YF, int ACT>
-__global__ __launch_bounds__(TPB) void k_gn_apply(const void* x, int x_f32, int x_ld, long long P, int C, int chunk,
+__global__ __launch_bounds__(TPB, GN_WAVES) void k_gn_apply(const void* x, int x_f32, int x_ld, long long P, int C, int chunk,
                                                   const crd_sum_t* stats, int gmul, const float* gamma, const float* beta,
                                                   int act, const float* mask, void* y, int y_ld, int y_f32, float y_inv_scale,
                                                   void* y2, int y2_ld) {
@@ -133,17 +243,13 @@
   const int c0 = m.cg * 8;
   long long p0 = (long long)blockIdx.x * chunk, p1 = p0 + chunk;
   if (p1 > P) p1 = P;
-  long long p = p0 + m.pl;
-  float v[U][8];
-  auto load_batch = [&](long long q) {
-#pragma unroll
-    for (int u = 0; u < U; ++u) {
-      long long pp = q + (long long)u * m.PL;
-      if (pp >= p1) pp = p1 - 1;
-      load8t<XF>(x, ((long long)b * P + pp) * x_ld + c0, v[u]);
-    }
-  };
-  if (p < p1) load_batch(p);
+  const long long row0 = (long long)b * P + p0;
+  const int q = m.pl, n = (int)(p1 - p0);
+  constexpr int NU = gn_form_slots(U_APPLY, XF ? 32 : 16);
+  Gran<XF> xq[NU];
+  Walk xw(x, XF ? 4 : 2, row0, x_ld, c0, m.pl, m.PL);
+  auto request = [&](int u) __attribute__((always_inline)) { xq[u].load(xw.next()); };
+  stream_first<NU>(q, n, m.PL, request);
   float ga[8], be[8], mk[8];
   load8(gamma, c0, 1, ga);
   load8(beta, c0, 1, be);
@@ -160,31 +266,23 @@
     ga[j] *= rstd;
     be[j] -= mean * ga[j];
   }
-  for (bool first = true; p < p1; p += (long long)U * m.PL, first = false) {
-    if (!first) load_batch(p);
-#pragma unroll
-    for (int u = 0; u < U; ++u) {
-      const long long pp = p + (long long)u * m.PL;
-      if (pp < p1) {
-#pragma unroll
-        for (int j = 0; j < 8; ++j) {
-          float w = v[u][j] * ga[j] + be[j];
-          if (ACT == 1) w = gelu_exact(w);
-          v[u][j] = w * mk[j];
-        }
-        if (YF == 3) {
-          store8_fp8(y, ((long long)b * P + pp) * y_ld + c0, v[u], y_inv_scale);
-          store8_bf16(y2, ((long long)b * P + pp) * y2_ld + c0, v[u]);
-        } else if (YF == 2) store8_fp8(y, ((long long)b * P + pp) * y_ld + c0, v[u], y_inv_scale);
-        else if (YF) store8_f32(reinterpret_cast<float*>(y), ((long long)b * P + pp) * y_ld + c0, v[u]);
-        else store8_bf16(y, ((long long)b * P + pp) * y_ld + c0, v[u]);
-      }
-    }
-  }
+  float v[8];
+  Walk yw(y, YF >= 2 ? 1 : YF ? 4 : 2, row0, y_ld, c0, m.pl, m.PL);
+  Walk y2w(y2, 2, row0, YF == 3 ? y2_ld : 0, c0, m.pl, m.PL);
+  stream_pixels<NU>(
+      q, n, m.PL, request, [&](int u) __attribute__((always_inline)) { xq[u].get(v); },
+      [&]() __attribute__((always_inline)) {
+#pragma unroll
+        for (int j = 0; j < 8; ++j) v[j] = gn_fwd_elem<ACT>(v[j], ga[j], be[j], mk[j]);
+        if (YF >= 2) store8_fp8(yw.next(), 0, v, y_inv_scale);
+        else if (YF) store8_f32(reinterpret_cast<float*>(yw.next()), 0, v);
+        else store8_bf16(yw.next(), 0, v);
+        if (YF == 3) store8_bf16(y2w.next(), 0, v);
+      });
 }
 
 template <int XF, int DF, int ACT>
-__global__ __launch_bounds__(TPB) void k_gn_bwd_reduce(const void* x, int x_f32, int x_ld, const void* dy, int dy_f32,
+__global__ __launch_bounds__(TPB, GN_WAVES) void k_gn_bwd_reduce(const void* x, int x_f32, int x_ld, const void* dy, int dy_f32,
                                                        int dy_ld, long long P, int C, int Cs, int chunk, const crd_sum_t* stats,
                                                        int gmul, const float* gamma, const float* beta, int act,
                                                        const float* mask, crd_sum_t* r, float* partial) {
@@ -195,18 +293,17 @@
     const int c0 = cs + m.cg * 8;
     long long p0 = (long long)blockIdx.x * chunk, p1 = p0 + chunk;
     if (p1 > P) p1 = P;
-    long long p = p0 + m.pl;
-    float v[U][8], d[U][8];
-    auto load_batch = [&](long long q) {
-#pragma unroll
-      for (int u = 0; u < U; ++u) {
-        long long pp = q + (long long)u * m.PL;
-        if (pp >= p1) pp = p1 - 1;
-        load8t<XF>(x, ((long long)b * P + pp) * x_ld + c0, v[u]);
-        load8t<DF>(dy, ((long long)b * P + pp) * dy_ld + c0, d[u]);
-      }
+    const long long row0 = (long long)b * P + p0;
+    const int q = m.pl, n = (int)(p1 - p0);
+    constexpr int NU = (XF && DF && ACT) ? 1 : gn_form_slots(U_RED, (XF ? 32 : 16) + (DF ? 32 : 16));
+    Gran<XF> xq[NU];
+    Gran<DF> dq[NU];
+    Walk xw(x, XF ? 4 : 2, row0, x_ld, c0, m.pl, m.PL), dw(dy, DF ? 4 : 2, row0, dy_ld, c0, m.pl, m.PL);
+    auto request = [&](int u) __attribute__((always_inline)) {
+      xq[u].load(xw.next());
+      dq[u].load(dw.next());
     };
-    if (p < p1) load_batch(p);
+    stream_first<NU>(q, n, m.PL, request);
     float ga[8], be[8], mk[8], s0[8], s1[8];
     load8(gamma, c0, 1, ga);
     load8(beta, c0, 1, be);
@@ -219,20 +316,20 @@
     float mean, rstd;
     const int grp = (c0 >> 4) / gmul;
     gn_mean_rstd(stats + (long long)b * (C >> 4) * 2, grp * gmul, gmul, (float)P * 16.f * gmul, mean, rstd);
-    for (bool first = true; p < p1; p += (long long)U * m.PL, first = false) {
-      if (!first) load_batch(p);
-#pragma unroll
-      for (int u = 0; u < U; ++u)
-        if (p + (long long)u * m.PL < p1) {
+    float v[8], d[8];
+    stream_pixels<NU>(
+        q, n, m.PL, request, [&](int u) __attribute__((always_inline)) { xq[u].get(v); dq[u].get(d); },
+        [&]() __attribute__((always_inline)) {
 #pragma unroll
           for (int j = 0; j < 8; ++j) {
-            float xh = (v[u][j] - mean) * rstd;
-            float g = d[u][j] * mk[j];
-            if (ACT == 1) g *= gelu_grad(xh * ga[j] + be[j]);
+            const float xh = gn_xhat(v[j], mean, rstd);
+            const float g = gn_bwd_g<ACT>(xh, d[j], ga[j], be[j], mk[j]);
             s0[j] += g; s1[j] += g * xh;
+            if (ACT == 1 && j == 3) __builtin_amdgcn_sched_barrier(0);
           }
-        }
-    }
+#pragma unroll
+          for (int j = 0; j < 8; ++j) asm volatile("" : "+v"(s0[j]), "+v"(s1[j]));
+        });
     float4* row = reinterpret_cast<float4*>(sm + (long long)m.pl * 2 * Cs + m.cg * 16);
 #pragma unroll
     for (int j = 0; j < 4; ++j) row[j] = make_float4(s0[2 * j], s1[2 * j], s0[2 * j + 1], s1[2 * j + 1]);
@@ -292,115 +389,112 @@
   }
 }
 
-template <int XF, int DF, int ACT>
-__global__ __launch_bounds__(TPB) void k_gn_bwd_apply(const void* x, int x_f32, int x_ld, const void* dy, int dy_f32,
-                                                      int dy_ld, long long P, int C, int chunk, const crd_sum_t* stats,
-                                                      int gmul, const float* gamma, const float* beta, int act,
-                                                      const float* mask, const crd_sum_t* r, float* dgamma, float* dbeta,
-                                                      void* dx, int dx_f32, int dx_ld, int dx_acc, int B, void* dx2, int dx2_ld,
-                                                      const float* scale2, unsigned char* dx8, int dx8_ld, const float* scale8,
-                                                      unsigned* amax8) {
-  const int b = blockIdx.y;
+struct BapArgs {
+  const void *x, *dy;
+  const crd_sum_t *stats, *r;
+  const float *gamma, *beta, *mask, *scale2, *scale8;
+  float *dgamma, *dbeta;
+  void *dx, *dx2;
+  unsigned char* dx8;
+  unsigned* amax8;
+  long long P;
+  int x_ld, dy_ld, dx_ld, dx2_ld, dx8_ld, C, chunk, gmul, B;
+};
+
+template <int XF, int DF, int ACT, int DXF, int ACC, int DX2, int FP8>
+__global__ __launch_bounds__(TPB, GN_WAVES) void k_gn_bwd_apply(const BapArgs a) {
+  const int b = blockIdx.y, C = a.C;
+  const long long P = a.P;
   Map m(C);
-  const int c0 = m.cg * 8;
-  __shared__ float s_amax[TPB / 64];
-  const float inv8 = (dx8 && scale8) ? 1.f / fmaxf(*scale8, 1e-30f) : 0.f;
   float amax = 0.f;
-  long long p0 = (long long)blockIdx.x * chunk, p1 = p0 + chunk;
-  if (p1 > P) p1 = P;
-  long long p = p0 + m.pl;
-  float v[U][8], d[U][8];
-  auto load_batch = [&](long long q) {
-#pragma unroll
-    for (int u = 0; u < U; ++u) {
-      long long pp = q + (long long)u * m.PL;
-      if (pp >= p1) pp = p1 - 1;
-      load8t<XF>(x, ((long long)b * P + pp) * x_ld + c0, v[u]);
-      load8t<DF>(dy, ((long long)b * P + pp) * dy_ld + c0, d[u]);
-    }
-  };
-  if (m.active && p < p1) load_batch(p);
-  if (b == 0 && dgamma) {
+  if (m.active) {
+    const int c0 = m.cg * 8;
+    long long p0 = (long long)blockIdx.x * a.chunk, p1 = p0 + a.chunk;
+    if (p1 > P) p1 = P;
+    const long long row0 = (long long)b * P + p0;
+    const int q = m.pl, n = (int)(p1 - p0);
+    constexpr int NU = gn_form_slots(U_BWD, (XF ? 32 : 16) + (DF ? 32 : 16) + (ACC ? (DXF ? 32 : 16) : 0));
+    Gran<XF> xq[NU];
+    Gran<DF> dq[NU];
+    Gran<DXF> wq[ACC ? NU : 1];
+    Walk xw(a.x, XF ? 4 : 2, row0, a.x_ld, c0, m.pl, m.PL), dw(a.dy, DF ? 4 : 2, row0, a.dy_ld, c0, m.pl, m.PL);
+    Walk ow(a.dx, DXF ? 4 : 2, row0, a.dx_ld, c0, m.pl, m.PL), aw = ow;
+    Walk o8w(a.dx8, 1, row0, FP8 ? a.dx8_ld : 0, c0, m.pl, m.PL), o2w(a.dx2, 2, row0, DX2 ? a.dx2_ld : 0, c0, m.pl, m.PL);
+    auto request = [&](int u) __attribute__((always_inline)) {
+      xq[u].load(xw.next());
+      dq[u].load(dw.next());
+      if (ACC) wq[u].load(aw.next());
+    };
+    stream_first<NU>(q, n, m.PL, request);
+    float ga[8], be[8], mk[8];
+    load8(a.gamma, c0, 1, ga);
+    load8(a.beta, c0, 1, be);
+    if (a.mask) load8(a.mask, (long long)b * C + c0, 1, mk);
+    else {
+#pragma unroll
+      for (int j = 0; j < 8; ++j) mk[j] = 1.f;
+    }
+    const int grp = (c0 >> 4) / a.gmul;
+    const int cpg = 16 * a.gmul;
+    const float inv_m = 1.f / ((float)P * cpg);
+    const crd_sum_t* rg = a.r + (long long)a.B * C * 2 + ((long long)b * (C / cpg) + grp) * 2;
+    const float S1 = grad_get(rg) * inv_m, S2 = grad_get(rg + 1) * inv_m;
+    float mean, rstd;
+    gn_mean_rstd(a.stats + (long long)b * (C >> 4) * 2, grp * a.gmul, a.gmul, (float)P * cpg, mean, rstd);
+    const float sc2 = (DX2 && a.scale2) ? a.scale2[b] : 1.f;
+    const float inv8 = (FP8 && a.scale8) ? 1.f / fmaxf(*a.scale8, 1e-30f) : 0.f;
+    float v[8], d[8], w[8];
+    stream_pixels<NU>(
+        q, n, m.PL, request,
+        [&](int u) __attribute__((always_inline)) {
+          xq[u].get(v); dq[u].get(d);
+          if (ACC) wq[u].get(w);
+        },
+        [&]() __attribute__((always_inline)) {
+          float o[8];
+#pragma unroll
+          for (int j = 0; j < 8; ++j) {
+            const float xh = gn_xhat(v[j], mean, rstd);
+            const float g = gn_bwd_g<ACT>(xh, d[j], ga[j], be[j], mk[j]);
+            o[j] = gn_bwd_dx(xh, g, ga[j], S1, S2, rstd);
+            if (ACT == 1 && j == 3) __builtin_amdgcn_sched_barrier(0);
+          }
+          if (ACC) {
+#pragma unroll
+            for (int j = 0; j < 8; ++j) o[j] = add_rounded(o[j], w[j]);
+          }
+          if (DXF) store8_f32(reinterpret_cast<float*>(ow.next()), 0, o);
+          else store8_bf16(ow.next(), 0, o);
+          if (FP8) {
+            const uint32_t w0 = pack_bf2(o[0], o[1]), w1 = pack_bf2(o[2], o[3]), w2 = pack_bf2(o[4], o[5]), w3 = pack_bf2(o[6], o[7]);
+            const float r[8] = {bf_lo(w0), bf_hi(w0), bf_lo(w1), bf_hi(w1), bf_lo(w2), bf_hi(w2), bf_lo(w3), bf_hi(w3)};
+            const float chk = ((r[0] + r[1]) + (r[2] + r[3])) + ((r[4] + r[5]) + (r[6] + r[7]));
+            if (!(fabsf(chk) < 3.0e38f)) crd_tu_nonfinite = 1;
+#pragma unroll
+            for (int j = 0; j < 8; ++j) amax = fmaxf(amax, fabsf(r[j]));
+            uint2 q8;
+            q8.x = pack_fp8x4(r[0] * inv8, r[1] * inv8, r[2] * inv8, r[3] * inv8);
+            q8.y = pack_fp8x4(r[4] * inv8, r[5] * inv8, r[6] * inv8, r[7] * inv8);
+            *reinterpret_cast<uint2*>(o8w.next()) = q8;
+          }
+          if (DX2) {
+#pragma unroll
+            for (int j = 0; j < 8; ++j) o[j] *= sc2;
+            store8_bf16(o2w.next(), 0, o);
+          }
+        });
+  }
+  if (b == 0 && a.dgamma) {
     for (int c = blockIdx.x * TPB + threadIdx.x; c < C; c += gridDim.x * TPB) {
-      const float ob = dbeta[c], og = dgamma[c];
+      const float ob = a.dbeta[c], og = a.dgamma[c];
       long long g0, g1;
-      sum_samples(r, B, C, c, g0, g1);
-      dbeta[c] = ob + (float)g0 * (1.f / GRAD_ONE);
-      dgamma[c] = og + (float)g1 * (1.f / GRAD_ONE);
-    }
-  }
-  if (!m.active && !amax8) return;
-  if (m.active) {
-  float ga[8], be[8], mk[8];
-  load8(gamma, c0, 1, ga);
-  load8(beta, c0, 1, be);
-  if (mask) load8(mask, (long long)b * C + c0, 1, mk);
-  else {
-#pragma unroll
-    for (int j = 0; j < 8; ++j) mk[j] = 1.f;
-  }
-  const int grp = (c0 >> 4) / gmul;
-  const int cpg = 16 * gmul;
-  const float inv_m = 1.f / ((float)P * cpg);
-  const crd_sum_t* rg = r + (long long)B * C * 2 + ((long long)b * (C / cpg) + grp) * 2;
-  const float S1 = grad_get(rg) * inv_m, S2 = grad_get(rg + 1) * inv_m;
-  float mean, rstd;
-  gn_mean_rstd(stats + (long long)b * (C >> 4) * 2, grp * gmul, gmul, (float)P * cpg, mean, rstd);
-  const float sc2 = (dx2 && scale2) ? scale2[b] : 1.f;
-  for (bool first = true; p < p1; p += (long long)U * m.PL, first = false) {
-    if (!first) load_batch(p);
-#pragma unroll
-    for (int u = 0; u < U; ++u) {
-      const long long pp = p + (long long)u * m.PL;
-      if (pp >= p1) continue;
-      float o[8];
-#pragma unroll
-      for (int j = 0; j < 8; ++j) {
-        float xh = (v[u][j] - mean) * rstd;
-        float g = d[u][j] * mk[j];
-        if (ACT == 1) g *= gelu_grad(xh * ga[j] + be[j]);
-        o[j] = (ga[j] * g - S1 - xh * S2) * rstd;
-      }
-      const long long off = ((long long)b * P + pp) * dx_ld + c0;
-      if (dx_f32) {
-        float* q = reinterpret_cast<float*>(dx);
-        if (dx_acc) {
-          float w[8];
-          load8(dx, off, 1, w);
-#pragma unroll
-          for (int j = 0; j < 8; ++j) o[j] += w[j];
-        }
-        store8_f32(q, off, o);
-      } else {
-        if (dx_acc) {
-          float w[8];
-          load8(dx, off, 0, w);
-#pragma unroll
-          for (int j = 0; j < 8; ++j) o[j] += w[j];
-        }
-        store8_bf16(dx, off, o);
-      }
-      if (dx8) {
-        const uint32_t w0 = pack_bf2(o[0], o[1]), w1 = pack_bf2(o[2], o[3]), w2 = pack_bf2(o[4], o[5]), w3 = pack_bf2(o[6], o[7]);
-        const float r[8] = {bf_lo(w0), bf_hi(w0), bf_lo(w1), bf_hi(w1), bf_lo(w2), bf_hi(w2), bf_lo(w3), bf_hi(w3)};
-        const float chk = ((r[0] + r[1]) + (r[2] + r[3])) + ((r[4] + r[5]) + (r[6] + r[7]));
-        if (!(fabsf(chk) < 3.0e38f)) crd_tu_nonfinite = 1;
-#pragma unroll
-        for (int j = 0; j < 8; ++j) amax = fmaxf(amax, fabsf(r[j]));
-        uint2 q8;
-        q8.x = pack_fp8x4(r[0] * inv8, r[1] * inv8, r[2] * inv8, r[3] * inv8);
-        q8.y = pack_fp8x4(r[4] * inv8, r[5] * inv8, r[6] * inv8, r[7] * inv8);
-        *reinterpret_cast<uint2*>(dx8 + ((long long)b * P + pp) * dx8_ld + c0) = q8;
-      }
-      if (dx2) {
-#pragma unroll
-        for (int j = 0; j < 8; ++j) o[j] *= sc2;
-        store8_bf16(dx2, ((long long)b * P + pp) * dx2_ld + c0, o);
-      }
-    }
-  }
-  }
-  if (amax8) {
+      sum_samples(a.r, a.B, C, c, g0, g1);
+      a.dbeta[c] = ob + (float)g0 * (1.f / GRAD_ONE);
+      a.dgamma[c] = og + (float)g1 * (1.f / GRAD_ONE);
+    }
+  }
+  if (FP8) {
+    __shared__ float s_amax[TPB / 64];
 #pragma unroll
     for (int o_ = 32; o_ > 0; o_ >>= 1) amax = fmaxf(amax, __shfl_xor(amax, o_));
     if ((threadIdx.x & 63) == 0) s_amax[threadIdx.x >> 6] = amax;
@@ -408,32 +502,71 @@
     if (threadIdx.x == 0) {
       float a_ = s_amax[0];
       for (int w_ = 1; w_ < TPB / 64; ++w_) a_ = fmaxf(a_, s_amax[w_]);
-      if (a_ > 0.f) atomicMax(amax8 + ((blockIdx.x + blockIdx.y * gridDim.x) % CRD_FP8_AMAX_SLOTS), __float_as_uint(a_));
-    }
-  }
-}
-
-inline void grid_for(long long P, int C, int B, dim3& grid, int& chunk, bool reduce = false) {
+      if (a_ > 0.f) atomicMax(a.amax8 + ((blockIdx.x + blockIdx.y * gridDim.x) % CRD_FP8_AMAX_SLOTS), __float_as_uint(a_));
+    }
+  }
+}
+
+struct GnKnobs { int minpix, small, cap_r, cap_e; };
+inline const GnKnobs& gn_knobs() {
+  static const GnKnobs k = {crd_dev_int("CRD_GN_MINPIX", 2), crd_dev_int("CRD_GN_SMALL", 256), crd_dev_int("CRD_GN_CAP_R", 768),
+                            crd_dev_int("CRD_GN_CAP_E", 2048)};
+  return k;
+}
+
+inline void grid_for(long long P, int C, int B, dim3& grid, int& chunk) {
+  const GnKnobs& k = gn_knobs();
   int CG = C >> 3;
   int PL = TPB / CG; if (PL < 1) PL = 1;
   long long per_block = (long long)PL * 8;
   long long nblk = (P + per_block - 1) / per_block;
-  static int minpix = -1, small = 256;
-  if (minpix < 0) {
-    minpix = crd_dev_int("CRD_GN_MINPIX", 2);
-    small = crd_dev_int("CRD_GN_SMALL", 256);
-  }
-  if (nblk * B < small && minpix < 8) {
-    per_block = (long long)PL * minpix;
+  if (nblk * B < k.small && k.minpix < 8) {
+    per_block = (long long)PL * k.minpix;
     nblk = (P + per_block - 1) / per_block;
   }
-  static int cap_r = -1, cap_e = -1;
-  if (cap_r < 0) { cap_r = crd_dev_int("CRD_GN_CAP_R", 768); cap_e = crd_dev_int("CRD_GN_CAP_E", 4096); }
-  long long cap = (reduce ? cap_r : cap_e) / (B > 0 ? B : 1); if (cap < 1) cap = 1;
+  long long cap = k.cap_r / (B > 0 ? B : 1); if (cap < 1) cap = 1;
   if (nblk > cap) nblk = cap;
   if (nblk < 1) nblk = 1;
   chunk = (int)((P + nblk - 1) / nblk);
   nblk = (P + chunk - 1) / chunk;
+  grid = dim3((unsigned)nblk, (unsigned)B);
+}
+
+inline int gn_slots(int kind) { return kind == 0 ? U_APPLY : U_BWD; }
+inline void gn_elem_shape(long long P, int C, int B, int kind, long long& nblk, long long& chunk, long long& batch) {
+  const GnKnobs& k = gn_knobs();
+  const int U_ = gn_slots(kind);
+  int CG = C >> 3;
+  int PL = TPB / CG; if (PL < 1) PL = 1;
+  batch = (long long)U_ * PL;
+  long long cap = k.cap_e / (B > 0 ? B : 1); if (cap < 1) cap = 1;
+  const long long per_block = (long long)PL * 8;
+  if ((P + per_block - 1) / per_block * B < k.small && k.minpix < 8) {
+    const long long pb = (long long)PL * k.minpix;
+    nblk = (P + pb - 1) / pb;
+    if (nblk > cap) nblk = cap;
+    if (nblk < 1) nblk = 1;
+    chunk = (P + nblk - 1) / nblk;
+  } else {
+    const long long nbatch = (P + batch - 1) / batch;
+    long long per = (nbatch + cap - 1) / cap;
+    const long long least = (8 + U_ - 1) / U_;
+    if (per < least) per = least;
+    chunk = per * batch;
+    if (chunk > P) chunk = P;
+  }
+  if (chunk < 1) chunk = 1;
+  nblk = (P + chunk - 1) / chunk;
+  if (nblk < 1) nblk = 1;
+}
+inline bool gn_chunk_fits(int chunk, int ld) { return ((long long)chunk + TPB) * ld * 4 < (1ll << 31); }
+#define CRD_GN_CHUNK_FITS(name, chunk, ld) \
+  CRD_UNSUPPORTED(gn_chunk_fits(chunk, ld), name ": a workgroup's %d rows of %d elements span 2 GiB or more", chunk, ld)
+
+inline void grid_elem(long long P, int C, int B, int kind, dim3& grid, int& chunk) {
+  long long nblk, ch, batch;
+  gn_elem_shape(P, C, B, kind, nblk, ch, batch);
+  chunk = (int)ch;
   grid = dim3((unsigned)nblk, (unsigned)B);
 }
 
@@ -461,7 +594,7 @@
   int rc = check_common("crd_gn_stats", x_ld, x_coff, C, x_f32);
   if (rc) return rc;
   dim3 grid; int chunk;
-  grid_for(P, C, B, grid, chunk, true);
+  grid_for(P, C, B, grid, chunk);
   if (x_f32) hipLaunchKernelGGL(k_gn_stats<1>, grid, dim3(TPB), lds_rows(C), as_stream(stream), off_ptr(x, x_f32, x_coff),
                                 x_f32, x_ld, (long long)P, C, chunk, stats, chan_sums);
   else hipLaunchKernelGGL(k_gn_stats<0>, grid, dim3(TPB), lds_rows(C), as_stream(stream), off_ptr(x, x_f32, x_coff),
@@ -476,7 +609,7 @@
   int rc = check_common("crd_attn_out_residual_stats", C, 0, C, 1);
   if (rc) return rc;
   dim3 grid; int chunk;
-  grid_for(N, C, B, grid, chunk, true);
+  grid_for(N, C, B, grid, chunk);
   hipLaunchKernelGGL(k_attn_out_residual_stats, grid, dim3(TPB), lds_rows(C), as_stream(stream), x, u, S, bp, dp, (long long)N, C,
                      chunk, x1, stats);
   CRD_LAUNCH_CHECK("crd_attn_out_residual_stats");
@@ -492,7 +625,8 @@
   int rc = check_common("crd_gn_apply", x_ld, x_coff, C, x_f32);
   if (rc) return rc;
   dim3 grid; int chunk;
-  grid_for(P, C, B, grid, chunk);
+  grid_elem(P, C, B, 0, grid, chunk);
+  CRD_GN_CHUNK_FITS("crd_gn_apply", chunk, x_ld > y_ld ? x_ld : y_ld);
   void* yp = y_f32 ? (void*)(reinterpret_cast<float*>(y) + y_coff) : (void*)(reinterpret_cast<bf16_t*>(y) + y_coff);
 #define CRD_GN_APPLY(XF, YF, ACT)                                                                                        \
   hipLaunchKernelGGL((k_gn_apply<XF, YF, ACT>), grid, dim3(TPB), 0, as_stream(stream), off_ptr(x, x_f32, x_coff), x_f32, \
@@ -519,7 +653,8 @@
   int rc = check_common("crd_gn_apply_fp8", x_ld, x_coff, C, x_f32);
   if (rc) return rc;
   dim3 grid; int chunk;
-  grid_for(P, C, B, grid, chunk);
+  grid_elem(P, C, B, 0, grid, chunk);
+  CRD_GN_CHUNK_FITS("crd_gn_apply_fp8", chunk, (x_ld > y_ld ? x_ld : y_ld) > yb_ld ? (x_ld > y_ld ? x_ld : y_ld) : yb_ld);
   void* yp = reinterpret_cast<unsigned char*>(y_fp8) + y_coff;
   void* y2 = y_bf16 ? (void*)(reinterpret_cast<bf16_t*>(y_bf16) + yb_coff) : nullptr;
 #define CRD_GN_APPLY8(XF, YF, ACT)                                                                                       \
@@ -555,8 +690,9 @@
       if (C % s_ == 0 && (C / s_) % cpg == 0 && (C / s_) % 8 == 0 && C / s_ >= 64) { S = s_; break; }
   }
   const int Cs = C / S;
-  grid_for(P, Cs, B * S, grid, chunk, true);
+  grid_for(P, Cs, B * S, grid, chunk);
   grid = dim3(grid.x, (unsigned)B, (unsigned)S);
+  CRD_GN_CHUNK_FITS("crd_gn_bwd_reduce", chunk, x_ld > dy_ld ? x_ld : dy_ld);
   float* part = (scratch && (long long)B * grid.x * 2 * C <= scratch_capacity && grid.x > 1) ? scratch : nullptr;
 #define CRD_GN_RED(XF, DF, ACT)                                                                                              \
   hipLaunchKernelGGL((k_gn_bwd_reduce<XF, DF, ACT>), grid, dim3(TPB), lds_rows(Cs), as_stream(stream),                     \
@@ -574,6 +710,21 @@
                        gamma, r, B);
   CRD_LAUNCH_CHECK("crd_gn_bwd_reduce");
   return CRD_OK;
+}
+
+constexpr int BAP_FORMS = 9, BAP_KEYS = 8 * BAP_FORMS;
+typedef void (*bap_launch_t)(dim3, hipStream_t, const BapArgs&);
+template <int K>
+static void bap_launch(dim3 grid, hipStream_t stream, const BapArgs& a) {
+  constexpr int F = K >> 3, F8 = F == 8;
+  hipLaunchKernelGGL((k_gn_bwd_apply<K & 1, (K >> 1) & 1, (K >> 2) & 1, F8 ? 0 : (F & 1), F8 ? 0 : ((F >> 1) & 1),
+                                     F8 ? 0 : ((F >> 2) & 1), F8>),
+                     grid, dim3(TPB), 0, stream, a);
+}
+template <int... K>
+static bap_launch_t bap_pick(int key, std::integer_sequence<int, K...>) {
+  static const bap_launch_t tab[] = {bap_launch<K>...};
+  return tab[key];
 }
 
 static int gn_bwd_apply_impl(const void* x, int32_t x_f32, int32_t x_ld, int32_t x_coff, const void* dy, int32_t dy_f32,
@@ -592,21 +743,40 @@
   int rc = check_common("crd_gn_bwd_apply", x_ld, x_coff, C, x_f32);
   if (rc) return rc;
   dim3 grid; int chunk;
-  grid_for(P, C, B, grid, chunk);
-  void* dxp = dx_f32 ? (void*)(reinterpret_cast<float*>(dx) + dx_coff) : (void*)(reinterpret_cast<bf16_t*>(dx) + dx_coff);
-#define CRD_GN_BAP(XF, DF, ACT)                                                                                              \
-  hipLaunchKernelGGL((k_gn_bwd_apply<XF, DF, ACT>), grid, dim3(TPB), 0, as_stream(stream), off_ptr(x, x_f32, x_coff), x_f32, \
-                     x_ld, off_ptr(dy, dy_f32, dy_coff), dy_f32, dy_ld, (long long)P, C, chunk, stats, gmul, gamma, beta,  \
-                     act, mask, r, dgamma, dbeta, dxp, dx_f32, dx_ld, dx_accumulate, B, dx2, dx2_ld, scale2, dx8p, dx8_ld, scale8,  \
-                     amax8)
-  switch ((x_f32 ? 4 : 0) | (dy_f32 ? 2 : 0) | (act ? 1 : 0)) {
-    case 0: CRD_GN_BAP(0, 0, 0); break;  case 1: CRD_GN_BAP(0, 0, 1); break;
-    case 2: CRD_GN_BAP(0, 1, 0); break;  case 3: CRD_GN_BAP(0, 1, 1); break;
-    case 4: CRD_GN_BAP(1, 0, 0); break;  case 5: CRD_GN_BAP(1, 0, 1); break;
-    case 6: CRD_GN_BAP(1, 1, 0); break;  default: CRD_GN_BAP(1, 1, 1); break;
-  }
-#undef CRD_GN_BAP
+  grid_elem(P, C, B, 1, grid, chunk);
+  {
+    int ld = x_ld > dy_ld ? x_ld : dy_ld;
+    if (dx_ld > ld) ld = dx_ld;
+    if (dx2 && dx2_ld > ld) ld = dx2_ld;
+    if (dx8 && dx8_ld > ld) ld = dx8_ld;
+    CRD_GN_CHUNK_FITS("crd_gn_bwd_apply", chunk, ld);
+  }
+  BapArgs a;
+  a.x = off_ptr(x, x_f32, x_coff); a.dy = off_ptr(dy, dy_f32, dy_coff);
+  a.stats = stats; a.r = r;
+  a.gamma = gamma; a.beta = beta; a.mask = mask; a.scale2 = scale2; a.scale8 = scale8;
+  a.dgamma = dgamma; a.dbeta = dbeta;
+  a.dx = dx_f32 ? (void*)(reinterpret_cast<float*>(dx) + dx_coff) : (void*)(reinterpret_cast<bf16_t*>(dx) + dx_coff);
+  a.dx2 = dx2; a.dx8 = dx8p; a.amax8 = amax8;
+  a.P = P;
+  a.x_ld = x_ld; a.dy_ld = dy_ld; a.dx_ld = dx_ld; a.dx2_ld = dx2_ld; a.dx8_ld = dx8_ld;
+  a.C = C; a.chunk = chunk; a.gmul = gmul; a.B = B;
+  const int form = dx8p ? 8 : ((dx_f32 ? 1 : 0) | (dx_accumulate ? 2 : 0) | (dx2 ? 4 : 0));
+  const int key = (x_f32 ? 1 : 0) | (dy_f32 ? 2 : 0) | (act ? 4 : 0) | (form << 3);
+  bap_pick(key, std::make_integer_sequence<int, BAP_KEYS>())(grid, as_stream(stream), a);
   CRD_LAUNCH_CHECK("crd_gn_bwd_apply");
+  return CRD_OK;
+}
+
+extern "C" int crd_gn_launch_shape(int32_t P, int32_t C, int32_t B, int32_t kind, int32_t* nblk, int32_t* chunk,
+                                   int32_t* batch_pixels) {
+  CRD_CHECK_ARG(nblk && chunk && batch_pixels, "crd_gn_launch_shape: null pointer");
+  CRD_CHECK_ARG(P >= 1 && B >= 1 && (kind == 0 || kind == 1), "crd_gn_launch_shape: P, B >= 1 and kind 0 (apply) or 1 (backward apply)");
+  int rc = check_common("crd_gn_launch_shape", 0, 0, C, 0);
+  if (rc) return rc;
+  long long n, ch, bp;
+  gn_elem_shape(P, C, B, kind, n, ch, bp);
+  *nblk = (int32_t)n; *chunk = (int32_t)ch; *batch_pixels = (int32_t)bp;
   return CRD_OK;
 }
 
diff --git a/camradepth_amd/lib.py b/camradepth_amd/lib.py
--- a/camradepth_amd/lib.py
+++ b/camradepth_amd/lib.py
@@ -131,6 +131,7 @@
     "crd_fp8_scale_update": "ppifip", "crd_quant_fp8_dev": "pliiipiipp", "crd_tune_conv3x3_small_grid": "i", "crd_tune_igemm_reg_epilogue": "i", "crd_conv_wgrad": "pp", "crd_conv_wgrad_splits": "p", "crd_conv_wgrad_route": "ppi", "crd_wgrad_group_build": "piplp", "crd_conv_wgrad_grouped": "ppp",
     "crd_gn_stats": "piiiiiippp", "crd_gn_apply": "piiiiiipippipPiiip".replace("P", "p"),
     "crd_gn_bwd_reduce": "piiipiiiiiipippippplp", "crd_gn_bwd_apply": "piiipiiiiiipippipppppiiiipipp",
+    "crd_gn_launch_shape": "iiiippp",
     "crd_dwconv3x3": "piiiippipppippppppp", "crd_dwconv3x3_wgrad": "ppiiiipipippp",
     "crd_attn_scores": "ppiiiiifppp", "crd_attn_scores_fp8": "ppiiiiffppp", "crd_attn_fwd": "ppiiiiifpppppppppp", "crd_attn_xbar": "ppppiiipp", "crd_attn_xbar_proj": "pppppiiippp", "crd_attn_vec_bwd": "ppiiifppp", "crd_attn_out_residual": "pppppiiipp", "crd_attn_out_residual_stats": "pppppiiippp",
     "crd_attn_out_bwd": "ppppiiipppp", "crd_attn_out_bwd_blocks": "iii", "crd_attn_out_bwd_gn": "ppppiiippppppppppp", "crd_attn_scores_bwd": "ppppiiiiifpppp", "crd_attn_bwd": "ppppiiiiifpppppifppp", "crd_attn_scores_bwd_partials": "iiiii", "crd_sum_partials_bf16": "pilplp", "crd_gsum_to_bf16": "pplp",
@@ -225,6 +226,13 @@
     return buf.value.decode()
 
 
+def gn_launch_shape(P, Cn, B, kind):
+    out = (C.c_int32 * 3)()
+    ptr = [C.cast(C.byref(out, 4 * i), C.c_void_p) for i in range(3)]
+    check(load().crd_gn_launch_shape(P, Cn, B, kind, *ptr), "crd_gn_launch_shape")
+    return out[0], out[1], out[2]
+
+
 def stream():
     return C.c_void_p(torch.cuda.current_stream().cuda_stream)
 
diff --git a/include/camradepth_hip.h b/include/camradepth_hip.h
--- a/include/camradepth_hip.h
+++ b/include/camradepth_hip.h
@@ -154,6 +154,7 @@
                      const crd_sum_t* r, float* dgamma, float* dbeta, void* dx, int32_t dx_f32, int32_t dx_ld,
                      int32_t dx_coff, int32_t dx_accumulate, void* dx2, int32_t dx2_ld, const float* scale2,
                      crd_stream_t stream);
+int crd_gn_launch_shape(int32_t P, int32_t C, int32_t B, int32_t kind, int32_t* nblk, int32_t* chunk, int32_t* batch_pixels);
 
 
 int crd_dwconv3x3(const void* x, int32_t B, int32_t H, int32_t W, int32_t C, const float* w9, const float* bias,
```
